# JKc66/CircuitVision

Hardware: AMD Instinct MI355X
Metric: circuit images/sec (YOLOv11 640² + SAM2.1-L 1024²) at 1/2/4/8 MI355X (higher is better)
Workload: dtype f16; 1 GPU; YOLO11-n 640x640 batch=32 f16 forward+decode+NMS (BASELINE configs[1]) + SAM2.1 Hiera-L 1024x1024 2 x batch=16 f16 learned-prompt wrapper forward (configs[2]) on the same images, per GPU and step; nc=62, weights=seeded random (SAM: LoRA merged), streams=3

## Files before the change

circuitvision_amd/_lib.py:

```python
import ctypes as C
import os

_HERE = os.path.dirname(os.path.abspath(__file__))
LIB_PATH = os.environ.get("CVMI_LIB_PATH") or os.path.join(_HERE, "libcvmi355.so")

F16, F32, BF16 = 0, 1, 2
ACT_NONE, ACT_SILU, ACT_RELU, ACT_GELU, ACT_SIGMOID = 0, 1, 2, 3, 4


class CvmiError(RuntimeError):
    pass


class ConvDesc(C.Structure):
    _fields_ = [
        ("x0", C.c_void_p), ("x1", C.c_void_p), ("w", C.c_void_p), ("bias", C.c_void_p),
        ("res", C.c_void_p), ("y", C.c_void_p),
        ("x0_ld", C.c_int), ("x1_ld", C.c_int), ("res_ld", C.c_int), ("y_ld", C.c_int),
        ("c0", C.c_int), ("c1", C.c_int), ("up0", C.c_int), ("up1", C.c_int),
        ("B", C.c_int), ("H", C.c_int), ("W", C.c_int), ("OH", C.c_int), ("OW", C.c_int),
        ("KH", C.c_int), ("KW", C.c_int), ("stride", C.c_int), ("pad", C.c_int),
        ("N", C.c_int), ("Kpad", C.c_int), ("act", C.c_int), ("dtype", C.c_int),
        ("out_f32", C.c_int), ("scalar_gather", C.c_int),
        ("res_mod", C.c_int), ("act_after_res", C.c_int), ("shuffle_cout", C.c_int), ("res_rep", C.c_int),
        ("row_stats", C.c_void_p),
    ]


class C3k2Desc(C.Structure):
    _fields_ = [
        ("x", C.c_void_p), ("y", C.c_void_p),
        ("w0", C.c_void_p), ("w1", C.c_void_p), ("w2", C.c_void_p), ("w3", C.c_void_p),
        ("b0", C.c_void_p), ("b1", C.c_void_p), ("b2", C.c_void_p), ("b3", C.c_void_p),
        ("x_ld", C.c_int), ("y_ld", C.c_int), ("kpad0", C.c_int), ("kpad1", C.c_int), ("kpad2", C.c_int), ("kpad3", C.c_int),
        ("B", C.c_int), ("H", C.c_int), ("W", C.c_int), ("c1", C.c_int), ("c", C.c_int), ("h", C.c_int), ("c2", C.c_int),
        ("fuse_cv1", C.c_int), ("shortcut", C.c_int), ("dtype", C.c_int),
    ]


class DwPwDesc(C.Structure):
    _fields_ = [
        ("x", C.c_void_p), ("y", C.c_void_p), ("wd", C.c_void_p), ("bd", C.c_void_p),
        ("w1", C.c_void_p), ("b1", C.c_void_p), ("w2", C.c_void_p), ("b2", C.c_void_p),
        ("x_ld", C.c_int), ("y_ld", C.c_int), ("kpad1", C.c_int), ("kpad2", C.c_int),
        ("B", C.c_int), ("H", C.c_int), ("W", C.c_int), ("C", C.c_int), ("N1", C.c_int), ("N2", C.c_int),
        ("dtype", C.c_int),
    ]


class AttnDesc(C.Structure):
    _fields_ = [
        ("q", C.c_void_p), ("k", C.c_void_p), ("v", C.c_void_p), ("o", C.c_void_p),
        ("q_sb", C.c_longlong), ("q_sh", C.c_longlong), ("q_st", C.c_longlong),
        ("k_sb", C.c_longlong), ("k_sh", C.c_longlong), ("k_st", C.c_longlong),
        ("v_sb", C.c_longlong), ("v_sh", C.c_longlong), ("v_st", C.c_longlong),
        ("o_sb", C.c_longlong), ("o_sh", C.c_longlong), ("o_st", C.c_longlong),
        ("B", C.c_int), ("heads", C.c_int), ("Nq", C.c_int), ("Nk", C.c_int),
        ("dqk", C.c_int), ("dv", C.c_int), ("scale", C.c_float), ("dtype", C.c_int),
        ("win", C.c_int), ("grid_h", C.c_int), ("grid_w", C.c_int), ("q_pool", C.c_int),
        ("q_bdiv", C.c_int), ("kv_bdiv", C.c_int), ("av_fp8", C.c_int), ("q_log2", C.c_int),
        ("proj_x", C.c_void_p), ("proj_w", C.c_void_p), ("proj_gamma", C.c_void_p), ("proj_beta", C.c_void_p), ("proj_stats", C.c_void_p),
        ("proj_ld", C.c_int), ("proj_K", C.c_int), ("proj_eps", C.c_float),
    ]


class LetterboxRow(C.Structure):
    _fields_ = [("src_byte_offset", C.c_longlong), ("H", C.c_int), ("W", C.c_int), ("new_h", C.c_int), ("new_w", C.c_int), ("top", C.c_int), ("left", C.c_int)]


class Sam2SrcRow(C.Structure):
    _fields_ = [("src_byte_offset", C.c_longlong), ("H", C.c_int), ("W", C.c_int), ("x0", C.c_int), ("y0", C.c_int), ("w", C.c_int), ("h", C.c_int)]


LETTERBOX_ROW = [(n, "<i8" if t is C.c_longlong else "<i4") for n, t in LetterboxRow._fields_]
SAM2_SRC_ROW = [(n, "<i8" if t is C.c_longlong else "<i4") for n, t in Sam2SrcRow._fields_]


_vp, _i, _f = C.c_void_p, C.c_int, C.c_float
SIGNATURES = {
    "cvmi_version": (_i, []),
    "cvmi_last_error": (C.c_char_p, []),
    "cvmi_last_kernel": (C.c_char_p, []),
    "cvmi_device_info": (_i, [_i, C.POINTER(_i)]),
    "cvmi_desc_size": (C.c_size_t, [_i]),
    "cvmi_graph_begin": (_i, [_vp]),
    "cvmi_graph_end": (_i, [_vp, C.POINTER(_vp)]),
    "cvmi_graph_launch": (_i, [_vp, _vp]),
    "cvmi_graph_destroy": (_i, [_vp]),
    "cvmi_conv2d": (_i, [C.POINTER(ConvDesc), _vp]),
    "cvmi_c3k2_supported": (_i, [_i, _i, _i, _i, _i, _i]),
    "cvmi_c3k2": (_i, [C.POINTER(C3k2Desc), _vp]),
    "cvmi_stem2_supported": (_i, [_i, _i, _i]),
    "cvmi_stem2": (_i, [_vp, _i, _vp, _vp, _i, _vp, _vp, _i, _vp, _i, _i, _i, _i, _i, _i, _i, _vp]),
    "cvmi_dwpw_supported": (_i, [_i, _i, _i, _i]),
    "cvmi_dwpw": (_i, [C.POINTER(DwPwDesc), _vp]),
    "cvmi_dwconv3x3": (_i, [_vp, _i, _vp, _vp, _vp, _i, _vp, _i, _i, _i, _i, _i, _i, _i, _vp]),
    "cvmi_sppf_pool": (_i, [_vp, _i, _i, _i, _i, _i, _i, _vp]),
    "cvmi_attention": (_i, [C.POINTER(AttnDesc), _vp]),
    "cvmi_detect_decode": (_i, [C.POINTER(_vp), C.POINTER(_i), C.POINTER(_vp), C.POINTER(_i), C.POINTER(_i),
                                C.POINTER(_i), C.POINTER(_f), _i, _i, _i, _i, _vp, _vp, _vp, _i, _vp]),
    "cvmi_yolo_nms_best": (_i, [_vp, _vp, _vp, _i, _i, _i, _f, _f, _i, _f, _vp, _vp, _vp, _vp, _vp]),
    "cvmi_yolo_nms_workspace": (C.c_size_t, [_i, _i]),
    "cvmi_yolo_nms": (_i, [_vp, _i, _i, _i, _f, _f, _i, _f, _vp, _vp, _vp, _vp, _vp]),
    "cvmi_letterbox": (_i, [_vp, _i, _i, _vp, _i, _i, _i, _i, _i, _i, _i, _i, _vp]),
    "cvmi_letterbox_batch": (_i, [_vp, _i, _i, _i, _vp, C.c_longlong, _i, _i, _i, _i, _i, _i, _i, _i, _vp]),
    "cvmi_letterbox_ragged": (_i, [_vp, C.c_longlong, _vp, _i, _vp, C.c_longlong, _i, _i, _i, _i, _vp]),
    "cvmi_nchw_to_nhwc": (_i, [_vp, _i, _vp, _i, _i, _i, _i, _i, _i, _vp]),
    "cvmi_nhwc_to_nchw_f32": (_i, [_vp, _i, _i, _vp, _i, _i, _i, _i, _vp]),
    "cvmi_layernorm": (_i, [_vp, _i, _i, _vp, _vp, _vp, _i, _i, C.c_longlong, _i, _f, _i, _i, _i, _i, _i, _vp]),
    "cvmi_layernorm_dual": (_i, [_vp, _i, _vp, _vp, _vp, _i, _vp, _i, _i, C.c_longlong, _i, _f, _vp]),
    "cvmi_hiera_mlp_supported": (_i, [_i]),
    "cvmi_hiera_mlp_packed_bytes": (C.c_size_t, [_i]),
    "cvmi_hiera_mlp": (_i, [_vp, _i, _vp, _vp, _f, _vp, _vp, C.c_longlong, _i, _i, _vp]),
    "cvmi_hiera_mlp_stats": (_i, [_vp, _i, _vp, _vp, _f, _vp, _vp, C.c_longlong, _i, _i, _vp, _f, _vp]),
    "cvmi_tok_linear_supported": (_i, [_i]),
    "cvmi_tok_linear_packed_bytes": (C.c_size_t, [_i, _i]),
    "cvmi_tok_linear_format": (_i, [_i]),
    "cvmi_tok_linear_stats_parts": (_i, [C.c_longlong, _i, _i]),
    "cvmi_tok_linear": (_i, [_vp, _i, _i, _vp, _vp, _f, _vp, _vp, _i, _i, C.c_longlong, _i, _i, _i, _i, _vp]),
    "cvmi_tok_linear_stats": (_i, [_vp, _i, _i, _vp, _vp, _f, _vp, _vp, _i, _i, C.c_longlong, _i, _i, _i, _i, _vp, _i, _vp, _f, _vp]),
    "cvmi_tok_linear_pool_stats": (_i, [_vp, _i, _vp, _vp, _f, _vp, _vp, _i, _i, _i, _i, _i, _i, _i, _vp, _vp]),
    "cvmi_tok_linear_pool": (_i, [_vp, _i, _vp, _vp, _f, _vp, _vp, _i, _i, _i, _i, _i, _i, _i, _vp]),
    "cvmi_maxpool2x2": (_i, [_vp, _i, _vp, _i, _i, _i, _i, _i, _i, _vp]),
    "cvmi_space_to_depth4": (_i, [_vp, _vp, _i, _i, _i, _i, _vp]),
    "cvmi_cast": (_i, [_vp, _i, _i, _vp, _i, _i, C.c_longlong, _i, _vp]),
    "cvmi_prompt_tokens": (_i, [_vp, _vp, _vp, _vp, _vp, _f, _vp, _vp, _i, _i, _i, _i, _vp]),
    "cvmi_repeat_images": (_i, [_vp, _vp, C.c_longlong, _i, _i, _vp]),
    "cvmi_hyper_masks": (_i, [_vp, _i, _vp, _i, _i, _i, _vp, _vp, _i, _i, _f, _vp]),
    "cvmi_select_mask": (_i, [_vp, _vp, _vp, _i, _i, _f, _vp, _vp, _vp, _i, _i, _vp]),
    "cvmi_multimask_out": (_i, [_vp, _vp, _i, _vp, _vp, _i, _i, _vp]),
    "cvmi_mask_prompt_embed": (_i, [_vp, _vp, _vp, _vp, _vp, _i, _i, _i, _i, _vp]),
    "cvmi_bilinear_f32": (_i, [_vp, _i, _i, _i, _vp, _i, _i, _vp, _f, _vp]),
    "cvmi_mask_extent": (_i, [_vp, _i, _i, _i, _vp, _vp]),
    "cvmi_mask_postprocess": (_i, [_vp, _i, _i, _i, _i, _i, _f, _vp, _vp, _vp]),
    "cvmi_mask_postprocess_sizes": (_i, [_vp, _i, _i, _i, _vp, _f, _vp, _vp, _vp]),
    "cvmi_mask_cc_workspace": (C.c_size_t, [_i, _i, _i]),
    "cvmi_mask_components": (_i, [_vp, _i, _i, _i, _f, _vp, _vp, _vp, _vp]),
    "cvmi_mask_fill_small": (_i, [_vp, _i, _i, _i, _f, _f, _f, _vp, _vp, _vp]),
    "cvmi_node_prepare": (_i, [_vp, _i, _vp, _vp, _vp, _vp, _vp, _vp]),
    "cvmi_enhance_lines": (_i, [_vp, _i, _vp, _vp, _vp, _vp]),
    "cvmi_contours_workspace": (C.c_size_t, [_i, _vp]),
    "cvmi_external_contours": (_i, [_vp, _vp, _i, _vp, _i, _vp, C.c_size_t, _i, _i, _vp, _vp, _vp, _vp, _vp]),
    "cvmi_node_connect_workspace": (C.c_size_t, [_i, _i]),
    "cvmi_node_connect": (_i, [_vp, _vp, _i, _i, _vp, _i, _vp, _vp, _vp, C.c_size_t, _vp, _vp, _vp]),
    "cvmi_segment_circuit": (_i, [_vp, C.c_size_t, _i, _vp, _i, _vp, _vp, _vp, _vp, _vp]),
    "cvmi_contour_hits_workspace": (C.c_size_t, [_i, _i]),
    "cvmi_contour_hits": (_i, [_vp, _vp, _i, _i, _vp, _i, _vp, _vp, _vp, C.c_size_t, _vp, _vp]),
    "cvmi_upsample_refine": (_i, [_vp, _i, _i, _i, _vp, _i, _i, _vp, C.POINTER(_i), _i, _i, _vp]),
    "cvmi_sam2_transform": (_i, [_vp, _i, _i, _vp, _i, _i, _vp]),
    "cvmi_sam2_transform_batch": (_i, [_vp, _i, _i, _i, _vp, _i, _i, _i, _vp]),
    "cvmi_sam2_transform_rects": (_i, [_vp, C.c_longlong, _i, _i, _vp, _i, _vp, _i, _i, _i, _vp]),
    "cvmi_sam2_transform_rects_dev": (_i, [_vp, C.c_longlong, _i, _i, _vp, _i, _vp, _i, _i, _i, _vp]),
    "cvmi_sam2_transform_srcs": (_i, [_vp, C.c_longlong, _vp, _i, _vp, _i, _i, _i, _vp]),
    "cvmi_mask_postprocess_rects_dev": (_i, [_vp, _i, _i, _i, _vp, C.c_longlong, _f, _vp, _vp, _vp]),
    "cvmi_stage2_crop": (_i, [_vp, _vp, _i, _i, _i, _i, _f, _i, _i, C.c_double, _i, _vp, _i, _vp, _vp, _vp, _vp, _vp, _vp, _vp]),
}

_lib = None


def load():
    global _lib
    if _lib is not None:
        return _lib
    if not os.path.exists(LIB_PATH):
        raise CvmiError(
            f"{LIB_PATH} not found: build it with `python -c 'import __graft_entry__ as g; g.build()'` "
            "(or `make -C circuitvision_amd/csrc`).  There is no CPU fallback.")
    import torch
    lib = C.CDLL(LIB_PATH)
    for name, (res, args) in SIGNATURES.items():
        fn = getattr(lib, name)
        fn.restype = res
        fn.argtypes = args
    check_abi(lib)
    _lib = lib
    return lib


DESC_MIRRORS = {0: ConvDesc, 1: C3k2Desc, 2: DwPwDesc, 3: AttnDesc}


def check_abi(lib, mirrors=None):
    for kind, cls in (mirrors or DESC_MIRRORS).items():
        want = int(lib.cvmi_desc_size(kind))
        if want != C.sizeof(cls):
            raise CvmiError(f"ABI mismatch: {cls.__name__} is {C.sizeof(cls)} bytes in this binding but {want} bytes in {LIB_PATH} "
                            f"(cvmi_desc_size({kind})); rebuild the library or update the binding to include/cvmi355.h")


def check(rc, what=""):
    if rc != 0:
        msg = load().cvmi_last_error().decode("utf-8", "replace")
        raise CvmiError(f"{what or 'cvmi call'} failed: {msg}")
```

circuitvision_amd/csrc/hiera_mlp.hip:

```cpp
#include "tok_stream.hpp"
#include <stdlib.h>

namespace {

#ifdef CVMI_OPERAND_BF16
#define CVMI_MFMA_ASM "v_mfma_f32_32x32x16_bf16"
#else
#define CVMI_MFMA_ASM "v_mfma_f32_32x32x16_f16"
#endif

template <int N1, int NT> constexpr int stage_frag(int i) { return i < N1 ? 2 * NT + i : (i - N1 < NT ? 2 * (i - N1) : 2 * (i - N1 - NT) + 1); }

template <int I, int N, typename F> __device__ __forceinline__ void static_for(F&& f) {
  if constexpr (I < N) {
    f(std::integral_constant<int, I>{});
    static_for<I + 1, N>(f);
  }
}

template <int C, int VAR = 0> struct MlpCfg {
  static_assert((C == 144 && VAR == 1) || (C == 288 && (VAR == 0 || VAR == 2)), "the instances that are built");
  static constexpr int KS = C / 16;
  static constexpr int KS1 = KS + 1;
  static constexpr int NT = (C + 31) / 32;
  static constexpr int NCH = 4 * C / 32;
  static constexpr int FR = KS1 + 2 * NT;
  static constexpr int CHB = FR * 1024;
  static constexpr int NW = 4;
  static constexpr int WPS = VAR == 1 ? 2 : 1;
  static constexpr int SLOTS = 2;
  static constexpr int CNT = (FR + NW - 1) / NW;
  static constexpr int LDS = SLOTS * CHB + 1024;
};

template <int C, int VAR = 0>
__global__ __launch_bounds__((MlpCfg<C, VAR>::NW * 64), (MlpCfg<C, VAR>::WPS)) void hiera_mlp_kernel(float* __restrict__ x, int x_ld, const float* __restrict__ gamma,
                                                                                      const float* __restrict__ beta, float eps,
                                                                                      const char* __restrict__ wp, const float* __restrict__ b2,
                                                                                      long long rows, float* __restrict__ stats_out, float stats_eps) {
  using Cfg = MlpCfg<C, VAR>;
  constexpr int KS = Cfg::KS, KS1 = Cfg::KS1, NT = Cfg::NT, NCH = Cfg::NCH, FR = Cfg::FR, CHB = Cfg::CHB, NW = Cfg::NW, CNT = Cfg::CNT, SLOTS = Cfg::SLOTS;
  extern __shared__ __attribute__((aligned(16))) char smem[];
  const int tid = threadIdx.x, wv = __builtin_amdgcn_readfirstlane(tid >> 6), lane = tid & 63;
  const int lr = lane & 31, lh = lane >> 5;
  const long long row_raw = ((long long)blockIdx.x * NW + wv) * 32 + lr;
  const bool row_ok = row_raw < rows;
  float* const xr = x + (row_ok ? row_raw : rows - 1) * (long long)x_ld;

  auto issue_chunk = [&](int j) {
    const char* src = wp + (size_t)j * CHB + lane * 16;
    char* dst = smem + (j % SLOTS) * CHB;
#pragma unroll
    for (int f = 0; f < CNT; ++f) {
      const int fi = f * NW + wv;
      const bool real = fi < FR;
      __builtin_amdgcn_global_load_lds((const __attribute__((address_space(1))) void*)(src + (size_t)(real ? fi : 0) * 1024),
                                       (__attribute__((address_space(3))) void*)(real ? dst + fi * 1024 : smem + SLOTS * CHB), 16, 0, 0);
    }
  };
  auto issue_piece = [&](int st, int f) {
    const int lo = st < 0 ? 2 * NT : 0, hi = st == NCH - 1 ? 2 * NT : FR;
    const char* src = wp + ((long long)st * FR + KS1) * 1024 + lane * 16;
    char* dst = smem + ((st + SLOTS) % SLOTS) * CHB;
    const int fi = f * NW + wv;
    const bool real = fi >= lo && fi < hi;
    __builtin_amdgcn_global_load_lds((const __attribute__((address_space(1))) void*)(src + (long long)(real ? fi : lo) * 1024),
                                     (__attribute__((address_space(3))) void*)(real ? dst + fi * 1024 : smem + SLOTS * CHB), 16, 0, 0);
  };
  auto issue_stage = [&](int st) {
#pragma unroll
    for (int f = 0; f < CNT; ++f) issue_piece(st, f);
  };
  if constexpr (VAR == 2) {
#pragma unroll
    for (int st = -1; st < SLOTS - 1; ++st) issue_stage(st);
  } else {
#pragma unroll
    for (int j = 0; j < SLOTS - 1; ++j) issue_chunk(j);
  }

  u32x4 xn[KS1];
  {
    float v[KS][8];
    float s = 0.f;
#pragma unroll
    for (int k = 0; k < KS; ++k) {
      const f32x4 a = *reinterpret_cast<const f32x4*>(xr + 16 * k + 8 * lh), b = *reinterpret_cast<const f32x4*>(xr + 16 * k + 8 * lh + 4);
#pragma unroll
      for (int e = 0; e < 4; ++e) { v[k][e] = a[e]; v[k][4 + e] = b[e]; s += a[e] + b[e]; }
    }
    s += __shfl_xor(s, 32);
    const float mean = s / (float)C;
    float q = 0.f;
#pragma unroll
    for (int k = 0; k < KS; ++k)
#pragma unroll
      for (int e = 0; e < 8; ++e) { const float d = v[k][e] - mean; q += d * d; }
    q += __shfl_xor(q, 32);
    const float rstd = 1.0f / sqrtf(q / (float)C + eps);
#pragma unroll
    for (int k = 0; k < KS; ++k) {
      const float* gp = gamma + 16 * k + 8 * lh;
      const float* bp = beta + 16 * k + 8 * lh;
      const f32x4 g0 = *reinterpret_cast<const f32x4*>(gp), g1 = *reinterpret_cast<const f32x4*>(gp + 4);
      const f32x4 b0 = *reinterpret_cast<const f32x4*>(bp), b1 = *reinterpret_cast<const f32x4*>(bp + 4);
      f16x8 h;
#pragma unroll
      for (int e = 0; e < 4; ++e) {
        h[e] = (f16)((v[k][e] - mean) * rstd * g0[e] + b0[e]);
        h[4 + e] = (f16)((v[k][4 + e] - mean) * rstd * g1[e] + b1[e]);
      }
      xn[k] = __builtin_bit_cast(u32x4, h);
    }
    const u32x4 one = {lh == 0 ? CVMI_ONE16X2 : 0u, 0u, 0u, 0u};
    xn[KS] = one;
  }

  f32x16 yacc[NT];
#pragma unroll
  for (int t = 0; t < NT; ++t)
#pragma unroll
    for (int r = 0; r < 16; ++r) yacc[t][r] = 0.f;

  if constexpr (VAR == 2) {
    static_assert(SLOTS == 2, "two stages in LDS");
    constexpr int PF = 6;
    f32x16 hA, hB;
    u32x4 ring_[PF];
#pragma unroll
    for (int f = 0; f < PF; ++f) asm volatile("" : "=v"(ring_[f]));
#pragma unroll
    for (int k = 0; k < KS1; ++k) asm volatile("s_nop 1" : "+v"(xn[k]));
    GeluPk2Steps gs[4];
    u32x4 pfv[2] = {};
    uint32_t c1v = GeluPk2Steps::GELU_C1_H;
    asm volatile("" : "+v"(c1v));
    auto gelu_step = [&](f32x16& h, auto kc) {
      constexpr int k = decltype(kc)::value, c = k >> 2;
      GeluPk2Steps& g = gs[c];
      if constexpr ((k & 3) == 0) g.s0(h[4 * c], h[4 * c + 1], h[4 * c + 2], h[4 * c + 3]);
      else if constexpr ((k & 3) == 1) g.s1(c1v);
      else if constexpr ((k & 3) == 2) g.s2();
      else {
        g.s3();
        pfv[c >> 1][2 * (c & 1)] = g.ra;
        pfv[c >> 1][2 * (c & 1) + 1] = g.rb;
      }
    };
    auto iter = [&](auto mode_, int slot, f32x16& hin, f32x16& hout) {
      constexpr int MODE = decltype(mode_)::value;
      constexpr int N1 = MODE == 2 ? 0 : KS1, N2 = MODE == 0 ? 0 : 2 * NT, NF = N1 + N2;
      const unsigned lbase_ = (unsigned)(size_t)((const __attribute__((address_space(3))) char*)(smem + slot * CHB + lane * 16));
      static_for<0, PF>([&](auto fc) {
        constexpr int f = decltype(fc)::value;
        u32x4(&ring)[PF] = ring_;
        const unsigned lbase = lbase_;
        asm volatile("ds_read_b128 %0, %1 offset:%2" : "+v"(ring[f]) : "v"(lbase), "n"(stage_frag<N1, NT>(f) * 1024));
      });
      if constexpr (MODE != 0) asm volatile("" : "+v"(hin));
      static_for<0, NF>([&](auto ic) {
        constexpr int i = decltype(ic)::value;
        u32x4(&ring)[PF] = ring_;
        const unsigned lbase = lbase_;
        f32x16 &hi_ = hin, &ho_ = hout;
        u32x4(&pfw)[2] = pfv;
        u32x4(&xf)[KS1] = xn;
        f32x16(&ya)[NT] = yacc;
        constexpr int young = (NF - 1 - i) < (PF - 1) ? (NF - 1 - i) : (PF - 1);
        constexpr bool refill = i + PF < NF;
        constexpr int off = refill ? stage_frag<N1, NT>(i + PF) * 1024 : 0;
        if constexpr (i == N1 && MODE != 0) asm volatile("s_nop 1" : "+v"(pfw[0]));
        if constexpr (i == N1 + NT && MODE != 0) asm volatile("s_nop 1" : "+v"(pfw[1]));
#define CVMI_MLP_BLK(TAIL, ACCC, ACC, B)                                                                                                              \
  if constexpr (refill)                                                                                                                                \
    asm volatile("s_waitcnt lgkmcnt(%[n])\n\t" CVMI_MFMA_ASM " %[acc], %[a], %[b], " TAIL "\n\tds_read_b128 %[a], %[lb] offset:%[off]"               \
                 : [acc] ACCC(ACC), [a] "+v"(ring[i % PF]) : [b] "v"(B), [lb] "v"(lbase), [n] "n"(young), [off] "n"(off));                             \
  else                                                                                                                                                 \
    asm volatile("s_waitcnt lgkmcnt(%[n])\n\t" CVMI_MFMA_ASM " %[acc], %[a], %[b], " TAIL : [acc] ACCC(ACC), [a] "+v"(ring[i % PF]) : [b] "v"(B), [n] "n"(young))
        if constexpr (i < N1) {
          if constexpr (i == 0) { CVMI_MLP_BLK("0", "=&v", ho_, xf[i]); }
          else { CVMI_MLP_BLK("%[acc]", "+v", ho_, xf[i]); }
        } else {
          constexpr int t = (i - N1) % NT, s2 = (i - N1) / NT;
          CVMI_MLP_BLK("%[acc]", "+a", ya[t], pfw[s2]);
        }
#undef CVMI_MLP_BLK
        constexpr int SL = MODE == 1 ? N1 + NT : NT, K0 = MODE == 1 ? 0 : 8;
        if constexpr (MODE != 0 && i < SL)
          static_for<K0, 16>([&](auto kc) {
            if constexpr ((decltype(kc)::value - K0) * SL / (16 - K0) == i) gelu_step(hi_, kc);
          });
      });
    };
    asm volatile("s_waitcnt vmcnt(%0)" ::"n"((SLOTS - 1) * CNT) : "memory");
    __syncthreads();
    iter(std::integral_constant<int, 0>{}, SLOTS - 1, hA, hA);
    auto step = [&](auto mode, int j, f32x16& hin, f32x16& hout) {
      asm volatile("s_waitcnt vmcnt(0)" ::: "memory");
      __syncthreads();
      if (j + 1 < NCH) issue_stage(j + 1);
      iter(mode, j % SLOTS, hin, hout);
    };
    static_assert(NCH % 2 == 0, "pairs of iterations");
#pragma unroll 1
    for (int j = 0; j < NCH - 2; j += 2) {
      step(std::integral_constant<int, 1>{}, j, hA, hB);
      step(std::integral_constant<int, 1>{}, j + 1, hB, hA);
    }
    step(std::integral_constant<int, 1>{}, NCH - 2, hA, hB);
    {
      asm volatile("s_waitcnt vmcnt(0)" ::: "memory");
      __syncthreads();
      asm volatile("" : "+v"(hB));
      static_for<0, 8>([&](auto kc) { gelu_step(hB, kc); });
      iter(std::integral_constant<int, 2>{}, (NCH - 1) % SLOTS, hB, hB);
    }
#pragma unroll
    for (int t = 0; t < NT; ++t) asm volatile("s_nop 15" : "+a"(yacc[t]));
#pragma unroll
    for (int f = 0; f < PF; ++f) asm volatile("" ::"v"(ring_[f]));
  } else
#pragma unroll 1
  for (int j = 0; j < NCH; ++j) {
    asm volatile("s_waitcnt vmcnt(0)" ::: "memory");
    __syncthreads();
    if (j + SLOTS - 1 < NCH) issue_chunk(j + SLOTS - 1);
    const char* const buf = smem + (j % SLOTS) * CHB + lane * 16;
    constexpr int PF = 6;
    u32x4 ring[PF];
    const unsigned lbase = (unsigned)(size_t)((const __attribute__((address_space(3))) char*)buf);
#pragma unroll
    for (int f = 0; f < PF; ++f) asm volatile("ds_read_b128 %0, %1 offset:%2" : "=v"(ring[f]) : "v"(lbase), "i"(f * 1024));
    f32x16 hacc;
#pragma unroll
    for (int r = 0; r < 16; ++r) hacc[r] = 0.f;
    f16x8 pf[2];
#pragma unroll
    for (int f = 0; f < FR; ++f) {
      ring_wait(ring[f % PF], (FR - 1 - f) < (PF - 1) ? (FR - 1 - f) : (PF - 1));
      const f16x8 a = __builtin_bit_cast(f16x8, ring[f % PF]);
      if (f < KS1) {
        hacc = CVMI_MFMA_32X32X16(a, __builtin_bit_cast(f16x8, xn[f]), hacc, 0, 0, 0);
      } else {
        const int t = (f - KS1) >> 1, s2 = (f - KS1) & 1;
        yacc[t] = CVMI_MFMA_32X32X16(a, pf[s2], yacc[t], 0, 0, 0);
      }
      if (f + PF < FR) asm volatile("ds_read_b128 %0, %1 offset:%2" : "=v"(ring[f % PF]) : "v"(lbase), "i"((f + PF) * 1024));
      if (f == KS1 - 1) {
#pragma unroll
        for (int r = 0; r < 16; r += 2) {
          const f16x2 g2 = gelu_fast_pk(hacc[r], hacc[r + 1]);
          pf[r >> 3][r & 7] = g2[0];
          pf[r >> 3][(r & 7) + 1] = g2[1];
        }
      }
    }
  }

  ShiftedSums st;
  if (stats_out) {
    const float o0 = row_ok ? xr[0] + (yacc[0][0] + b2[0]) : 0.f;
    st.shift = __shfl(o0, lr);
  }
  if (row_ok) {
#pragma unroll
    for (int t = 0; t < NT; ++t)
#pragma unroll
      for (int g = 0; g < 4; ++g) {
        const int c0 = 32 * t + 8 * g + 4 * lh;
        if (c0 < C) {
          const f32x4 bb = *reinterpret_cast<const f32x4*>(b2 + c0);
          f32x4 o = *reinterpret_cast<const f32x4*>(xr + c0);
#pragma unroll
          for (int e = 0; e < 4; ++e) o[e] += yacc[t][4 * g + e] + bb[e];
          *reinterpret_cast<f32x4*>(xr + c0) = o;
          if (stats_out) st.add(o);
        }
      }
  }
  if (stats_out) {
    const float2 mr = shifted_mean_rstd(st.shift, row_sum<2>(st.s), row_sum<2>(st.q), (float)C, stats_eps);
    if (row_ok && lh == 0) *reinterpret_cast<float2*>(stats_out + 2 * row_raw) = mr;
  }
}

template <int C, int VAR = 0>
int launch_mlp(float* x, int x_ld, const float* gamma, const float* beta, float eps, const void* wp, const float* b2, long long rows, hipStream_t s,
               float* stats_out, float stats_eps) {
  using Cfg = MlpCfg<C, VAR>;
  static hipError_t attr = hipFuncSetAttribute(reinterpret_cast<const void*>(&hiera_mlp_kernel<C, VAR>), hipFuncAttributeMaxDynamicSharedMemorySize, Cfg::LDS);
  CVMI_HIP(attr);
  const long long per = (long long)Cfg::NW * 32;
  cvmi_note_kernel("hiera_mlp_kernel<%d, %d>", C, VAR);
  hipLaunchKernelGGL((hiera_mlp_kernel<C, VAR>), dim3((unsigned)((rows + per - 1) / per)), dim3(Cfg::NW * 64), Cfg::LDS, s, x, x_ld, gamma, beta, eps,
                     (const char*)wp, b2, rows, stats_out, stats_eps);
  CVMI_LAUNCH_CHECK();
  return 0;
}

}

#ifndef CVMI_OPERAND_BF16
extern "C" int cvmi_hiera_mlp_supported(int C) { return C == 144 || C == 288; }

extern "C" size_t cvmi_hiera_mlp_packed_bytes(int C) {
  if (!cvmi_hiera_mlp_supported(C)) return 0;
  const size_t fr = (size_t)(C / 16 + 1) + 2 * (size_t)((C + 31) / 32);
  return (size_t)(4 * C / 32) * fr * 1024;
}
extern "C" int cvmi_hiera_mlp_stats_bf16(void* x, int x_ld, const float* gamma, const float* beta, float eps, const void* w_packed, const float* b2,
                                         long long rows, int C, int dtype, float* ln_stats_out, float ln_stats_eps, cvmi_stream_t stream_);
#endif

extern "C" int CVMI_ENTRY(cvmi_hiera_mlp_stats)(void* x, int x_ld, const float* gamma, const float* beta, float eps, const void* w_packed, const float* b2,
                                                long long rows, int C, int dtype, float* ln_stats_out, float ln_stats_eps, cvmi_stream_t stream_) {
#ifndef CVMI_OPERAND_BF16
  if (dtype == CVMI_BF16) return cvmi_hiera_mlp_stats_bf16(x, x_ld, gamma, beta, eps, w_packed, b2, rows, C, dtype, ln_stats_out, ln_stats_eps, stream_);
#endif
  CVMI_CHECK(dtype == CVMI_T16, "hiera_mlp: dtype must be CVMI_F16 or CVMI_BF16");
  CVMI_CHECK(x && gamma && beta && w_packed && b2 && rows > 0, "hiera_mlp: bad arguments");
  CVMI_CHECK(C == 144 || C == 288, "hiera_mlp: C=%d is not built (144, 288)", C);
  CVMI_CHECK(x_ld >= C && x_ld % 4 == 0 && (((uintptr_t)x | (uintptr_t)gamma | (uintptr_t)beta | (uintptr_t)w_packed | (uintptr_t)b2) & 15) == 0 &&
                 ((uintptr_t)ln_stats_out & 7) == 0,
             "hiera_mlp: pointers / ld must be 16-byte aligned");
  hipStream_t s = (hipStream_t)stream_;
  float* xf = (float*)x;
  if (C == 144) return launch_mlp<144, 1>(xf, x_ld, gamma, beta, eps, w_packed, b2, rows, s, ln_stats_out, ln_stats_eps);
  const char* const pipe = getenv("CVMI_MLP_PIPE");
  if (pipe && !(atoi(pipe) & 2)) return launch_mlp<288, 0>(xf, x_ld, gamma, beta, eps, w_packed, b2, rows, s, ln_stats_out, ln_stats_eps);
  return launch_mlp<288, 2>(xf, x_ld, gamma, beta, eps, w_packed, b2, rows, s, ln_stats_out, ln_stats_eps);
}

extern "C" int CVMI_ENTRY(cvmi_hiera_mlp)(void* x, int x_ld, const float* gamma, const float* beta, float eps, const void* w_packed, const float* b2,
                                          long long rows, int C, int dtype, cvmi_stream_t stream_) {
  return CVMI_ENTRY(cvmi_hiera_mlp_stats)(x, x_ld, gamma, beta, eps, w_packed, b2, rows, C, dtype, nullptr, 0.f, stream_);
}
```

circuitvision_amd/engine.py:

```python
import ctypes as C
import os
import threading

import torch

from . import _lib
from ._lib import BF16, F16, F32, AttnDesc, C3k2Desc, ConvDesc

TORCH_DTYPE = {F16: torch.float16, F32: torch.float32, BF16: torch.bfloat16}
ESIZE = {F16: 2, F32: 4, BF16: 2}
DTYPE_OF = {torch.float16: F16, torch.float32: F32, torch.bfloat16: BF16}


def is16(dtype):
    return dtype in (F16, BF16)


def require_gpu():
    if not torch.cuda.is_available():
        raise _lib.CvmiError("circuitvision_amd needs an MI355X (gfx950) GPU: torch.cuda.is_available() is False; "
                             "there is no CPU fallback")
    _lib.load()


class Buf:

    def __init__(self, B, H, W, C, dtype, device="cuda", zero=False):
        self.B, self.H, self.W, self.C, self.dtype = B, H, W, C, dtype
        alloc = torch.zeros if zero else torch.empty
        self.t = alloc((B, H, W, C), dtype=TORCH_DTYPE[dtype], device=device)

    def view(self, c0=0, c=None):
        return View(self, c0, self.C - c0 if c is None else c)

    def images(self, b0, nb):
        assert 0 <= b0 and b0 + nb <= self.B
        o = Buf.__new__(Buf)
        o.B, o.H, o.W, o.C, o.dtype = nb, self.H, self.W, self.C, self.dtype
        o.t = self.t[b0:b0 + nb]
        return o

    @property
    def nbytes(self):
        return self.t.numel() * self.t.element_size()


class View:

    def __init__(self, buf, c0, c):
        assert 0 <= c0 and c0 + c <= buf.C, (c0, c, buf.C)
        self.buf, self.c0, self.c = buf, c0, c

    @property
    def ptr(self):
        return self.buf.t.data_ptr() + self.c0 * ESIZE[self.buf.dtype]

    @property
    def ld(self):
        return self.buf.C

    B = property(lambda s: s.buf.B)
    H = property(lambda s: s.buf.H)
    W = property(lambda s: s.buf.W)
    dtype = property(lambda s: s.buf.dtype)

    def tensor(self):
        return self.buf.t[..., self.c0:self.c0 + self.c]


class PackedConv:

    def __init__(self, weight, bias, dtype, device="cuda"):
        N, Cin, KH, KW = weight.shape
        K = Cin * KH * KW
        Npad = (N + 127) // 128 * 128
        Kpad = (K + 63) // 64 * 64
        w = torch.zeros(Npad, Kpad, dtype=torch.float32)
        w[:N, :K] = weight.permute(0, 2, 3, 1).reshape(N, K)
        b = torch.zeros(Npad, dtype=torch.float32)
        if bias is not None:
            b[:N] = bias
        self.w = w.to(TORCH_DTYPE[dtype]).to(device)
        self.bias = b.to(device)
        self.N, self.Cin, self.KH, self.KW, self.K, self.Kpad, self.dtype = N, Cin, KH, KW, K, Kpad, dtype
        self.param_bytes = N * K * ESIZE[dtype]


class PackedDW:

    def __init__(self, weight, bias, dtype, device="cuda"):
        C_ = weight.shape[0]
        assert weight.shape[1:] == (1, 3, 3)
        self.w = weight.reshape(C_, 9).t().contiguous().to(TORCH_DTYPE[dtype]).to(device)
        self.bias = (bias if bias is not None else torch.zeros(C_)).float().to(device)
        self.C, self.dtype = C_, dtype
        self.param_bytes = C_ * 9 * ESIZE[dtype]


class Plan:

    def __init__(self, stream):
        self.stream = stream
        self.ops = []
        self.keep = []
        self.graph = None
        self.lanes, self.cur_lane = [], 0
        self._lane_streams = {}
        self._lock = threading.Lock()

    @property
    def sptr(self):
        return self.stream.cuda_stream

    def add(self, label, kind, thunk, bytes_=0, flops=0):
        self.ops.append((label, kind, thunk, bytes_, flops))
        self.lanes.append(self.cur_lane)

    def fork(self):
        self.add("fork", "sync", lambda sp=None: None)
        self.lanes[-1] = -1

    def lane(self, i):
        self.cur_lane = i

    def join(self):
        self.cur_lane = 0
        self.add("join", "sync", lambda sp=None: None)
        self.lanes[-1] = -2

    def run_eager(self):
        for _, _, thunk, _, _ in self.ops:
            thunk()

    def capture(self):
        lib = _lib.load()
        self.run_eager()
        self.stream.synchronize()
        _lib.check(lib.cvmi_graph_begin(self.sptr), "graph_begin")
        try:
            self._run_lanes()
        finally:
            g = C.c_void_p()
            rc = lib.cvmi_graph_end(self.sptr, C.byref(g))
        _lib.check(rc, "graph_end")
        self.graph = g

    def _run_lanes(self):
        active, lane_fork = {}, {}
        for (label, kind, thunk, _, _), lane in zip(self.ops, self.lanes):
            if lane == -1:
                self._fork_ev = torch.cuda.Event()
                self._fork_ev.record(self.stream)
            elif lane == -2:
                for st in active.values():
                    ev = torch.cuda.Event()
                    ev.record(st)
                    self.stream.wait_event(ev)
                active, lane_fork = {}, {}
            elif lane == 0:
                thunk()
            else:
                if lane not in self._lane_streams:
                    self._lane_streams[lane] = torch.cuda.Stream(device=self.stream.device)
                st = self._lane_streams[lane]
                if lane_fork.get(lane) is not self._fork_ev:
                    st.wait_event(self._fork_ev)
                    lane_fork[lane] = self._fork_ev
                    active[lane] = st
                thunk(st.cuda_stream)

    def run(self):
        if self.graph is None:
            self.capture()
        _lib.check(_lib.load().cvmi_graph_launch(self.graph, self.sptr), "graph_launch")

    def timed_eager(self, with_kernels=False):
        lib = _lib.load()
        lib.cvmi_last_kernel()
        evs = []
        for label, kind, thunk, b, f in self.ops:
            e0 = torch.cuda.Event(enable_timing=True)
            e1 = torch.cuda.Event(enable_timing=True)
            e0.record(self.stream)
            thunk()
            e1.record(self.stream)
            evs.append((label, kind, e0, e1, b, f, lib.cvmi_last_kernel().decode()))
        self.stream.synchronize()
        if with_kernels:
            return [(l, k, e0.elapsed_time(e1), b, f, kn) for l, k, e0, e1, b, f, kn in evs]
        return [(l, k, e0.elapsed_time(e1), b, f) for l, k, e0, e1, b, f, _ in evs]

    def __del__(self):
        try:
            if self.graph is not None:
                if self._lane_streams or os.environ.get("CVMI_KEEP_GRAPHS") == "1":
                    _PARKED_GRAPHS.append((self.graph, self._lane_streams))
                else:
                    _lib.load().cvmi_graph_destroy(self.graph)
        except Exception:
            pass


_PARKED_GRAPHS = []


def row_stats_supported(M, N, K):
    if N % 192 or N < 384 or K < 1024 or K % 64:
        return False
    t256 = -(-M // 256) * -(-N // 256)
    if t256 >= 256 and N / (-(-N // 256) * 256) >= 0.8 and t256 / (-(-t256 // 256) * 256) >= 0.8:
        return False
    t192 = -(-M // 256) * (N // 192)
    return t192 >= 256 and t192 / (-(-t192 // 256) * 256) >= 0.75


def op_conv(plan, label, pc, srcs, dst, stride=1, pad=None, act=_lib.ACT_NONE, res=None, out_hw=None,
            scalar_gather=False, kind="conv", res_mod=0, act_after_res=False, shuffle_cout=0, res_rep=0, row_stats=None):
    lib = _lib.load()
    (v0, up0) = srcs[0]
    v1, up1 = (srcs[1] if len(srcs) > 1 else (None, 0))
    H, W = v0.H << up0, v0.W << up0
    if v1 is not None:
        assert (v1.H << up1, v1.W << up1) == (H, W), "concatenated sources disagree on size"
    ctot = v0.c + (v1.c if v1 is not None else 0)
    assert ctot == pc.Cin, (label, ctot, pc.Cin)
    pad = pc.KH // 2 if pad is None else pad
    OH = (H + 2 * pad - pc.KH) // stride + 1
    OW = (W + 2 * pad - pc.KW) // stride + 1
    if out_hw is not None:
        assert out_hw[0] <= OH and out_hw[1] <= OW
        OH, OW = out_hw
    if shuffle_cout:
        assert (dst.B, dst.H, dst.W) == (v0.B, 2 * OH, 2 * OW) and dst.c == shuffle_cout and pc.N == 4 * shuffle_cout, label
    else:
        assert (dst.B, dst.H, dst.W) == (v0.B, OH, OW) and dst.c == pc.N, (label, (dst.B, dst.H, dst.W, dst.c), (v0.B, OH, OW, pc.N))
    if res_rep > 1:
        assert res is not None and res.B * res_rep == v0.B, (label, "res_rep needs a per-image residual")
        assert shuffle_cout or res_mod == dst.H * dst.W, (label, "res_rep: ConvTranspose scatter or res_mod = rows per image")
    out_f32 = 1 if (dst.dtype == F32 and is16(pc.dtype)) else 0
    d = ConvDesc(
        x0=v0.ptr, x1=(v1.ptr if v1 is not None else None), w=pc.w.data_ptr(), bias=pc.bias.data_ptr(),
        res=(res.ptr if res is not None else None), y=dst.ptr,
        x0_ld=v0.ld, x1_ld=(v1.ld if v1 is not None else 0), res_ld=(res.ld if res is not None else 0), y_ld=dst.ld,
        c0=v0.c, c1=(v1.c if v1 is not None else 0), up0=up0, up1=up1,
        B=v0.B, H=H, W=W, OH=OH, OW=OW, KH=pc.KH, KW=pc.KW, stride=stride, pad=pad,
        N=pc.N, Kpad=pc.Kpad, act=act, dtype=pc.dtype, out_f32=out_f32, scalar_gather=1 if scalar_gather else 0,
        res_mod=res_mod, act_after_res=1 if act_after_res else 0, shuffle_cout=shuffle_cout, res_rep=res_rep,
        row_stats=(row_stats.data_ptr() if row_stats is not None else None))
    if row_stats is not None:
        assert row_stats.dtype == torch.float32 and row_stats.is_contiguous() and row_stats.numel() == v0.B * OH * OW * (pc.N // 96) * 2, label
    plan.keep.append((d, pc, srcs, dst, res, row_stats))
    sp0 = plan.sptr
    fn = lib.cvmi_conv2d

    def thunk(sp=None):
        sp = sp0 if sp is None else sp
        _lib.check(fn(C.byref(d), sp), label)

    M = v0.B * OH * OW
    es, oes = ESIZE[pc.dtype], ESIZE[dst.dtype]
    in_elems = v0.B * (v0.H * v0.W * v0.c + (v1.H * v1.W * v1.c if v1 is not None else 0))
    bytes_ = in_elems * es + M * pc.N * oes + (M * pc.N * oes if res is not None else 0)
    plan.add(label, kind, thunk, bytes_, 2 * M * pc.N * pc.K)
    return d


def c3k2_supported(c1, c, h, c2, fuse_cv1, dtype):
    return bool(_lib.load().cvmi_c3k2_supported(c1, c, h, c2, 1 if fuse_cv1 else 0, dtype))


def op_c3k2(plan, label, src, dst, pc_cv1, pc_m1, pc_m2, pc_cv2, c, h, fuse_cv1, shortcut=True):
    lib = _lib.load()
    assert (src.B, src.H, src.W) == (dst.B, dst.H, dst.W) and dst.c == pc_cv2.N
    assert src.c == (pc_cv1.Cin if fuse_cv1 else 2 * c), (label, src.c)
    d = C3k2Desc(x=src.ptr, y=dst.ptr, w0=pc_cv1.w.data_ptr() if fuse_cv1 else None, w1=pc_m1.w.data_ptr(), w2=pc_m2.w.data_ptr(),
                 w3=pc_cv2.w.data_ptr(), b0=pc_cv1.bias.data_ptr() if fuse_cv1 else None, b1=pc_m1.bias.data_ptr(), b2=pc_m2.bias.data_ptr(),
                 b3=pc_cv2.bias.data_ptr(), x_ld=src.ld, y_ld=dst.ld, kpad0=pc_cv1.Kpad if fuse_cv1 else 0, kpad1=pc_m1.Kpad, kpad2=pc_m2.Kpad,
                 kpad3=pc_cv2.Kpad, B=src.B, H=src.H, W=src.W, c1=pc_cv1.Cin if fuse_cv1 else 0, c=c, h=h, c2=pc_cv2.N,
                 fuse_cv1=1 if fuse_cv1 else 0, shortcut=1 if shortcut else 0, dtype=pc_cv2.dtype)
    plan.keep.append((d, src, dst, pc_cv1, pc_m1, pc_m2, pc_cv2))
    sp0, fn = plan.sptr, lib.cvmi_c3k2

    def thunk(sp=None):
        sp = sp0 if sp is None else sp
        _lib.check(fn(C.byref(d), sp), label)

    px = src.B * src.H * src.W
    flops = 2 * px * ((pc_cv1.Cin * 2 * c if fuse_cv1 else 0) + 9 * c * h * 2 + 3 * c * pc_cv2.N)
    plan.add(label, "conv", thunk, px * (src.c + dst.c) * ESIZE[pc_cv2.dtype], flops)


def stem2_supported(c0, c1, dtype):
    return bool(_lib.load().cvmi_stem2_supported(c0, c1, dtype))


def op_stem2(plan, label, pc0, pc1, src, dst):
    lib = _lib.load()
    assert src.c == 16 and pc0.Cin == 16 and pc1.Cin == pc0.N and dst.c == pc1.N
    assert (dst.H, dst.W) == ((src.H - 1) // 2 + 1, (src.W - 1) // 2 + 1) and dst.B == src.B
    args = (src.ptr, src.ld, pc0.w.data_ptr(), pc0.bias.data_ptr(), pc0.Kpad, pc1.w.data_ptr(), pc1.bias.data_ptr(), pc1.Kpad,
            dst.ptr, dst.ld, src.B, src.H, src.W, pc0.N, pc1.N, pc1.dtype)
    plan.keep.append((pc0, pc1, src, dst))
    sp0, fn = plan.sptr, lib.cvmi_stem2

    def thunk(sp=None):
        sp = sp0 if sp is None else sp
        _lib.check(fn(*args, sp), label)

    px0, px1 = src.B * src.H * src.W, dst.B * dst.H * dst.W
    plan.add(label, "stem", thunk, (px0 * src.c + px1 * dst.c) * ESIZE[pc1.dtype], 2 * px0 * 27 * pc0.N + 2 * px1 * 9 * pc0.N * pc1.N)


def dwpw_supported(C_, n1, n2, dtype):
    return bool(_lib.load().cvmi_dwpw_supported(C_, n1, n2, dtype))


def op_dwpw(plan, label, pd, pc1, src, dst, pc2=None):
    lib = _lib.load()
    assert src.c == pd.C == pc1.Cin and (src.B, src.H, src.W) == (dst.B, dst.H, dst.W)
    assert dst.c == (pc2.N if pc2 is not None else pc1.N) and (pc2 is None or pc2.Cin == pc1.N)
    d = _lib.DwPwDesc(x=src.ptr, y=dst.ptr, wd=pd.w.data_ptr(), bd=pd.bias.data_ptr(), w1=pc1.w.data_ptr(), b1=pc1.bias.data_ptr(),
                      w2=pc2.w.data_ptr() if pc2 is not None else None, b2=pc2.bias.data_ptr() if pc2 is not None else None,
                      x_ld=src.ld, y_ld=dst.ld, kpad1=pc1.Kpad, kpad2=pc2.Kpad if pc2 is not None else 0,
                      B=src.B, H=src.H, W=src.W, C=pd.C, N1=pc1.N, N2=pc2.N if pc2 is not None else 0, dtype=pc1.dtype)
    plan.keep.append((d, pd, pc1, pc2, src, dst))
    sp0, fn = plan.sptr, lib.cvmi_dwpw

    def thunk(sp=None):
        sp = sp0 if sp is None else sp
        _lib.check(fn(C.byref(d), sp), label)

    px = src.B * src.H * src.W
    flops = px * (18 * pd.C + 2 * pd.C * pc1.N + (2 * pc1.N * pc2.N if pc2 is not None else 0))
    plan.add(label, "head", thunk, px * (src.c + dst.c) * ESIZE[pc1.dtype], flops)


def op_dwconv(plan, label, pd, src, dst, act=_lib.ACT_NONE, res=None):
    lib = _lib.load()
    assert src.c == pd.C == dst.c and (src.B, src.H, src.W) == (dst.B, dst.H, dst.W)
    args = (src.ptr, src.ld, pd.w.data_ptr(), pd.bias.data_ptr(), res.ptr if res is not None else None,
            res.ld if res is not None else 0, dst.ptr, dst.ld, src.B, src.H, src.W, pd.C, act, pd.dtype)
    plan.keep.append((pd, src, dst, res))
    sp0 = plan.sptr
    fn = lib.cvmi_dwconv3x3

    def thunk(sp=None):
        sp = sp0 if sp is None else sp
        _lib.check(fn(*args, sp), label)

    n = src.B * src.H * src.W * pd.C
    plan.add(label, "dwconv", thunk, n * ESIZE[pd.dtype] * (3 if res is not None else 2), 18 * n)


def op_sppf_pool(plan, label, buf, c):
    lib = _lib.load()
    args = (buf.t.data_ptr(), buf.C, buf.B, buf.H, buf.W, c, buf.dtype)
    plan.keep.append(buf)
    sp0 = plan.sptr
    fn = lib.cvmi_sppf_pool

    def thunk(sp=None):
        sp = sp0 if sp is None else sp
        _lib.check(fn(*args, sp), label)

    n = buf.B * buf.H * buf.W * c
    plan.add(label, "pool", thunk, 4 * n * ESIZE[buf.dtype], 0)


def op_attention(plan, label, desc, keep, bytes_=0, flops=0):
    lib = _lib.load()
    plan.keep.append((desc, keep))
    sp0 = plan.sptr
    fn = lib.cvmi_attention

    def thunk(sp=None):
        sp = sp0 if sp is None else sp
        _lib.check(fn(C.byref(desc), sp), label)

    plan.add(label, "attention", thunk, bytes_, flops)


def make_attn_desc(**kw):
    d = AttnDesc()
    for k, v in kw.items():
        setattr(d, k, v)
    return d


class Rows:

    def __init__(self, t, rows, C, ld=None, offset=0, dtype=None):
        self.t, self.rows, self.C = t, rows, C
        self.ld = ld if ld is not None else C
        self.offset = offset
        self.dtype = dtype if dtype is not None else DTYPE_OF[t.dtype]

    @property
    def ptr(self):
        return self.t.data_ptr() + self.offset * self.t.element_size()


def op_layernorm(plan, label, src, gamma, beta, dst, eps=1e-6, act=_lib.ACT_NONE, pad=None, dst2=None):
    lib = _lib.load()
    src, dst = _as_rows(src), _as_rows(dst)
    assert src.C == dst.C == gamma.numel()
    if dst2 is not None:
        dst2 = _as_rows(dst2)
        assert pad is None and act == _lib.ACT_NONE and src.dtype == dst.dtype == _lib.F32 and is16(dst2.dtype)
        assert dst2.rows == src.rows and dst2.C == src.C
        args2 = (src.ptr, src.ld, gamma.data_ptr(), beta.data_ptr(), dst.ptr, dst.ld, dst2.ptr, dst2.ld, dst2.dtype, src.rows, src.C, float(eps))
        plan.keep.append((src, dst, dst2, gamma, beta))
        sp1, fn2 = plan.sptr, lib.cvmi_layernorm_dual

        def thunk2(sp=None):
            sp = sp1 if sp is None else sp
            _lib.check(fn2(*args2, sp), label)

        plan.add(label, "layernorm", thunk2, src.rows * src.C * (4 + 4 + 2), 8 * src.rows * src.C)
        return
    if pad is None:
        assert src.rows == dst.rows
        pad = (0, 0, 0, 0)
    else:
        assert src.rows % (pad[0] * pad[1]) == 0 and dst.rows == src.rows // (pad[0] * pad[1]) * pad[2] * pad[3]
    args = (src.ptr, src.ld, src.dtype, gamma.data_ptr(), beta.data_ptr(), dst.ptr, dst.ld, dst.dtype, src.rows, src.C, float(eps), act) + tuple(pad)
    plan.keep.append((src, dst, gamma, beta))
    sp0, fn = plan.sptr, lib.cvmi_layernorm

    def thunk(sp=None):
        sp = sp0 if sp is None else sp
        _lib.check(fn(*args, sp), label)

    plan.add(label, "layernorm", thunk, src.rows * src.C * (ESIZE[src.dtype] + ESIZE[dst.dtype]), 8 * src.rows * src.C)


def _as_rows(v):
    if isinstance(v, Rows):
        return v
    if isinstance(v, View):
        return Rows(v.buf.t, v.B * v.H * v.W, v.c, ld=v.ld, offset=v.c0, dtype=v.dtype)
    raise TypeError(type(v))


def op_maxpool2(plan, label, src, dst):
    lib = _lib.load()
    assert src.c == dst.c and (dst.H, dst.W) == (src.H // 2, src.W // 2) and src.dtype == dst.dtype
    args = (src.ptr, src.ld, dst.ptr, dst.ld, src.B, src.H, src.W, src.c, src.dtype)
    plan.keep.append((src, dst))
    sp0, fn = plan.sptr, lib.cvmi_maxpool2x2

    def thunk(sp=None):
        sp = sp0 if sp is None else sp
        _lib.check(fn(*args, sp), label)

    n = src.B * src.H * src.W * src.c
    plan.add(label, "pool", thunk, n * ESIZE[src.dtype] * 5 // 4, 0)


def op_cast(plan, label, src, dst):
    lib = _lib.load()
    src, dst = _as_rows(src), _as_rows(dst)
    args = (src.ptr, src.ld, src.dtype, dst.ptr, dst.ld, dst.dtype, src.rows, src.C)
    plan.keep.append((src, dst))
    sp0, fn = plan.sptr, lib.cvmi_cast

    def thunk(sp=None):
        sp = sp0 if sp is None else sp
        _lib.check(fn(*args, sp), label)

    plan.add(label, "cast", thunk, src.rows * src.C * (ESIZE[src.dtype] + ESIZE[dst.dtype]), 0)


def op_call(plan, label, kind, fn, args, keep=(), bytes_=0, flops=0):
    plan.keep.append(keep)
    sp0 = plan.sptr

    def thunk(sp=None):
        sp = sp0 if sp is None else sp
        _lib.check(fn(*args, sp), label)

    plan.add(label, kind, thunk, bytes_, flops)


def hiera_mlp_supported(C_, dtype):
    return is16(dtype) and bool(_lib.load().cvmi_hiera_mlp_supported(C_))


class PackedHieraMlp:

    def __init__(self, w1, b1, w2, b2, device="cuda", dtype=F16):
        td = TORCH_DTYPE[dtype]
        Hd, C_ = w1.shape
        assert Hd == 4 * C_ and tuple(w2.shape) == (C_, Hd) and C_ % 16 == 0
        ks1, nt, nch = C_ // 16 + 1, (C_ + 31) // 32, Hd // 32
        b_hi = b1.to(td).float()
        b_lo = (b1 - b_hi).to(td).float()
        w1x = torch.cat((w1, b_hi[:, None], b_lo[:, None], torch.zeros(Hd, 14)), 1)
        f1 = w1x.view(nch, 32, ks1, 2, 8).permute(0, 2, 3, 1, 4)
        w2p = torch.zeros(nt * 32, Hd)
        w2p[:C_] = w2
        f2 = w2p.view(nt, 32, nch, 2, 2, 2, 4).permute(2, 0, 3, 5, 1, 4, 6)
        packed = torch.cat((f1.reshape(nch, -1), f2.reshape(nch, -1)), 1).contiguous()
        assert packed.numel() * 2 == _lib.load().cvmi_hiera_mlp_packed_bytes(C_)
        self.w = packed.to(td).to(device)
        self.bias = b2.float().contiguous().to(device)
        self.C, self.dtype = C_, dtype
        self.param_bytes = 2 * Hd * C_ * 2


def op_hiera_mlp(plan, label, pm, x, gamma, beta, eps=1e-6, stats_out=None, stats_eps=1e-6):
    lib = _lib.load()
    assert x.dtype == F32 and x.c == pm.C and x.c0 == 0
    rows = x.B * x.H * x.W
    assert stats_out is None or (stats_out.dtype == torch.float32 and stats_out.numel() == 2 * rows and stats_out.is_contiguous()), label
    args = (x.ptr, x.ld, gamma.data_ptr(), beta.data_ptr(), float(eps), pm.w.data_ptr(), pm.bias.data_ptr(), rows, pm.C, pm.dtype,
            stats_out.data_ptr() if stats_out is not None else None, float(stats_eps))
    plan.keep.append((pm, x, gamma, beta, stats_out))
    sp0, fn = plan.sptr, lib.cvmi_hiera_mlp_stats

    def thunk(sp=None):
        sp = sp0 if sp is None else sp
        _lib.check(fn(*args, sp), label)

    plan.add(label, "mlp_fused", thunk, rows * pm.C * 8, 2 * rows * 2 * 4 * pm.C * pm.C)


def tok_linear_supported(K, dtype, rows):
    return is16(dtype) and rows % 256 == 0 and bool(_lib.load().cvmi_tok_linear_supported(K))


class PackedTokLinear:

    def __init__(self, w, b, device="cuda", dtype=F16):
        N, K = w.shape
        td = TORCH_DTYPE[dtype]
        assert K % 16 == 0
        if _lib.load().cvmi_tok_linear_format(K) == 16:
            nch, ks = (N + 31) // 32, K // 32
            b = b if b is not None else torch.zeros(N)
            wx = torch.zeros(nch * 32, K)
            wx[:N] = w
            frag = wx.view(nch, 2, 16, ks, 4, 8).permute(0, 3, 1, 4, 2, 5).reshape(nch, ks * 2 * 512)
            bias = torch.zeros(nch * 32)
            bias[:N] = b
            piece = torch.zeros(nch, 512, dtype=torch.int16)
            piece[:, :64] = bias.view(nch, 32).contiguous().view(torch.int16)
            packed = torch.cat((frag.to(td).contiguous().view(torch.int16), piece), 1).contiguous()
            assert packed.numel() * 2 == _lib.load().cvmi_tok_linear_packed_bytes(K, N)
            self.w = packed.to(device)
            self.bias = torch.zeros(4, device=device)
            self.N, self.K, self.dtype = N, K, dtype
            self.param_bytes = N * K * 2
            return
        ks1, nch = K // 16 + 1, ((N + 31) // 32 + 1) // 2 * 2
        b = b if b is not None else torch.zeros(N)
        b_hi = b.to(td).float()
        b_lo = (b - b_hi).to(td).float()
        wx = torch.zeros(nch * 32, K + 16)
        wx[:N, :K], wx[:N, K], wx[:N, K + 1] = w, b_hi, b_lo
        packed = wx.view(nch, 32, ks1, 2, 8).permute(0, 2, 3, 1, 4).contiguous()
        assert packed.numel() * 2 == _lib.load().cvmi_tok_linear_packed_bytes(K, N)
        self.w = packed.to(td).to(device)
        self.bias = torch.zeros(4, device=device)
        self.N, self.K, self.dtype = N, K, dtype
        self.param_bytes = N * K * 2


def qkv_attn_rows(heads, hd=72):
    C_ = heads * hd
    rows = []
    for h in range(heads):
        for c in range(3):
            for r in range(32):
                g, lh, e = r >> 3, (r >> 2) & 1, r & 3
                d = 32 * c + 16 * (g >> 1) + 8 * lh + 4 * (g & 1) + e
                rows.append(h * hd + d if d < hd else -1)
        rows += [C_ + h * hd + n if n < hd else 2 * C_ + h * hd + n - hd if n < 2 * hd else -1 for n in range(160)]
    return rows


def qkv_attn_supported(dim, dout, heads, ws, q_pool, dtype, nwin):
    return is16(dtype) and dim == 144 and ws == 8 and nwin % 2 == 0 and (dout, heads) == ((288, 4) if q_pool else (144, 2))


class PackedQkvAttn:

    def __init__(self, w, b, heads, device="cuda", dtype=F16):
        N, K = w.shape
        assert N % (3 * heads) == 0
        self.rows = qkv_attn_rows(heads, N // (3 * heads))
        idx = torch.tensor(self.rows)
        keep = (idx >= 0).float()
        b = b if b is not None else torch.zeros(N)
        pt = PackedTokLinear(w[idx.clamp(min=0)] * keep[:, None], b[idx.clamp(min=0)] * keep, device, dtype)
        self.w, self.bias = pt.w, pt.bias
        self.N, self.K, self.heads, self.dtype = N, K, heads, dtype
        self.param_bytes = pt.param_bytes


def tok_linear_stats_parts(rows, K, N):
    return int(_lib.load().cvmi_tok_linear_stats_parts(rows, K, N))


def op_tok_linear(plan, label, pt, src, dst, ln=None, act=_lib.ACT_NONE, residual=False, kind="gemm", stats_in=None, stats_out=None, stats_eps=1e-6,
                  stats_parts=0):
    lib = _lib.load()
    src, dst = _as_rows(src), _as_rows(dst)
    assert src.C == pt.K and dst.C == pt.N and src.rows == dst.rows and src.rows % 256 == 0, label
    assert (src.dtype == F32) == (ln is not None) and (dst.dtype == F32) == bool(residual), label
    assert (ln is not None or src.dtype == pt.dtype) and (residual or dst.dtype == pt.dtype), label
    cast = isinstance(ln, str)
    assert not cast or ln == "cast", label
    assert stats_in is None or (ln is not None and not cast), label
    assert stats_out is None or residual, label
    out_parts = tok_linear_stats_parts(src.rows, pt.K, pt.N) if stats_out is not None else 0
    assert stats_out is None or (stats_out.dtype == torch.float32 and stats_out.numel() == 2 * src.rows * max(out_parts, 1) and stats_out.is_contiguous()), label
    assert stats_in is None or (stats_in.dtype == torch.float32 and stats_in.numel() == 2 * src.rows * max(stats_parts, 1) and stats_in.is_contiguous()), label
    gam, bet, eps = ln if (ln is not None and not cast) else (None, None, 0.0)
    args = (src.ptr, src.ld, 2 if cast else 1 if ln is not None else 0, gam.data_ptr() if gam is not None else None, bet.data_ptr() if bet is not None else None,
            float(eps), pt.w.data_ptr(), dst.ptr, dst.ld, 1 if residual else 0, src.rows, pt.K, pt.N, act, pt.dtype,
            stats_in.data_ptr() if stats_in is not None else None, int(stats_parts), stats_out.data_ptr() if stats_out is not None else None, float(stats_eps))
    plan.keep.append((pt, src, dst, gam, bet, stats_in, stats_out))
    sp0, fn = plan.sptr, lib.cvmi_tok_linear_stats

    def thunk(sp=None):
        sp = sp0 if sp is None else sp
        _lib.check(fn(*args, sp), label)

    bytes_ = src.rows * (pt.K * ESIZE[src.dtype] + pt.N * ESIZE[dst.dtype] * (2 if residual else 1))
    plan.add(label, kind, thunk, bytes_, 2 * src.rows * pt.N * pt.K)


def op_tok_linear_pool(plan, label, pt, src, dst, ln, kind="gemm", stats_in=None):
    lib = _lib.load()
    B, H, W = src.B, src.H, src.W
    assert src.dtype == F32 and dst.dtype == F32 and src.c == pt.K and dst.c == pt.N, label
    assert (dst.B, dst.H, dst.W) == (B, H // 2, W // 2) and H % 2 == 0 and W % 2 == 0 and (B * H * W) % 256 == 0, label
    gam, bet, eps = ln
    assert stats_in is None or (stats_in.dtype == torch.float32 and stats_in.numel() == 2 * B * H * W and stats_in.is_contiguous()), label
    args = (src.ptr, src.ld, gam.data_ptr(), bet.data_ptr(), float(eps), pt.w.data_ptr(), dst.ptr, dst.ld, B, H, W, pt.K, pt.N, pt.dtype,
            stats_in.data_ptr() if stats_in is not None else None)
    plan.keep.append((pt, src, dst, gam, bet, stats_in))
    sp0, fn = plan.sptr, lib.cvmi_tok_linear_pool_stats

    def thunk(sp=None):
        sp = sp0 if sp is None else sp
        _lib.check(fn(*args, sp), label)

    rows = B * H * W
    plan.add(label, kind, thunk, rows * pt.K * 4 + rows // 4 * pt.N * 4, 2 * rows * pt.N * pt.K)
```

circuitvision_amd/sam2.py:

```python
import hashlib
import math
import os
import threading

import numpy as np
import torch
import torch.nn.functional as TF

from . import _lib
from ._lib import ACT_GELU, ACT_NONE, ACT_RELU, ACT_SIGMOID, BF16, F16, F32
from .engine import (ESIZE, TORCH_DTYPE, is16, Buf, PackedConv, PackedHieraMlp, PackedQkvAttn, PackedTokLinear, Plan, Rows, hiera_mlp_supported, make_attn_desc, op_attention,
                     op_call, op_cast, op_conv, op_hiera_mlp, op_layernorm, op_maxpool2, op_tok_linear, op_tok_linear_pool, require_gpu, row_stats_supported,
                     qkv_attn_supported, tok_linear_stats_parts, tok_linear_supported)

LOG2E = 1.4426950408889634
HIERA_L = dict(embed_dim=144, num_heads=2, stages=(2, 6, 36, 4), global_att_blocks=(23, 33, 43), window_spec=(8, 4, 16, 8))
HIERA_T = dict(embed_dim=96, num_heads=1, stages=(1, 2, 7, 2), global_att_blocks=(5, 7, 9), window_spec=(8, 4, 14, 7))

LORA_TARGETS_REFERENCE = (
    [f"sam_mask_decoder.transformer.layers.{l}.{a}.{p}" for l in (0, 1) for a in ("self_attn", "cross_attn_token_to_image")
     for p in ("k_proj", "q_proj", "v_proj", "out_proj")]
    + [f"sam_mask_decoder.transformer.layers.{l}.mlp.layers.{j}" for l in (0, 1) for j in (0, 1)]
    + ["sam_mask_decoder.iou_prediction_head.layers.2", "sam_mask_decoder.conv_s0", "sam_mask_decoder.conv_s1",
       "image_encoder.neck.convs.2.conv", "image_encoder.neck.convs.3.conv",
       "image_encoder.trunk.blocks.44.attn.qkv", "image_encoder.trunk.blocks.44.mlp.layers.0", "image_encoder.trunk.blocks.44.proj",
       "image_encoder.trunk.blocks.47.attn.qkv", "image_encoder.trunk.blocks.47.mlp.layers.0"]
    + [f"sam_mask_decoder.transformer.layers.{l}.cross_attn_image_to_token.{p}" for l in (0, 1) for p in ("q_proj", "k_proj", "v_proj")])


MASK_DOWN = "sam_prompt_encoder.mask_downscaling"
MASK_DOWN_PARAMS = 4684


def mask_down_tensors():
    return [(f"{MASK_DOWN}.0.weight", (4, 1, 2, 2), "w"), (f"{MASK_DOWN}.0.bias", (4,), "w"),
            (f"{MASK_DOWN}.1.weight", (4,), "gamma"), (f"{MASK_DOWN}.1.bias", (4,), "w"),
            (f"{MASK_DOWN}.3.weight", (16, 4, 2, 2), "w"), (f"{MASK_DOWN}.3.bias", (16,), "w"),
            (f"{MASK_DOWN}.4.weight", (16,), "gamma"), (f"{MASK_DOWN}.4.bias", (16,), "w"),
            (f"{MASK_DOWN}.6.weight", (256, 16, 1, 1), "w"), (f"{MASK_DOWN}.6.bias", (256,), "w")]


class SamSyntheticParams:

    def __init__(self, seed=0, lora_targets=LORA_TARGETS_REFERENCE, r=4, alpha=16, std=0.02):
        self.seed, self.targets, self.r, self.scaling, self.std, self.sd = seed, set(lora_targets), r, alpha / r, std, {}
        self.mask_sd = {}

    def _t(self, name, shape, kind="w"):
        sd = self.mask_sd if name.startswith(MASK_DOWN + ".") else self.sd
        if name in sd:
            assert tuple(sd[name].shape) == tuple(shape), (name, sd[name].shape, shape)
            return sd[name]
        h = int.from_bytes(hashlib.sha256(f"{self.seed}:{name}".encode()).digest()[:8], "little") & 0x7FFFFFFFFFFFFFFF
        g = torch.Generator().manual_seed(h)
        if kind == "gamma":
            t = torch.empty(shape).uniform_(0.8, 1.2, generator=g)
        elif kind == "unit":
            t = torch.empty(shape).normal_(0, 1.0, generator=g)
        elif kind == "refine":
            t = torch.empty(shape).normal_(0, 0.2, generator=g)
        else:
            t = torch.empty(shape).normal_(0, self.std, generator=g).clamp_(-2 * self.std, 2 * self.std)
        sd[name] = t
        return t

    def weight(self, mod, shape):
        if mod in self.targets:
            w = self._t(f"{mod}.base_layer.weight", shape)
            a_shape = (self.r, shape[1]) + tuple(shape[2:])
            b_shape = (shape[0], self.r) + (1,) * (len(shape) - 2)
            A = self._t(f"{mod}.lora_A.default.weight", a_shape)
            Bm = self._t(f"{mod}.lora_B.default.weight", b_shape)
            delta = (Bm.reshape(shape[0], self.r) @ A.reshape(self.r, -1)).reshape(shape)
            return w + self.scaling * delta
        return self._t(f"{mod}.weight", shape)

    def bias(self, mod, n):
        return self._t(f"{mod}.base_layer.bias" if mod in self.targets else f"{mod}.bias", (n,))

    def tensor(self, name, shape, kind="w"):
        return self._t(name, shape, kind)

    def state_dict(self):
        return dict(self.sd)

    def mask_prompt_state_dict(self):
        for name, shape, kind in mask_down_tensors():
            self._t(name, shape, kind)
        return dict(self.mask_sd)


class SamBlankParams:

    def weight(self, mod, shape):
        return torch.zeros(shape)

    def bias(self, mod, n):
        return torch.zeros(n)

    def tensor(self, name, shape, kind="w"):
        return torch.zeros(shape)

    def state_dict(self):
        return {}


class SamStateDictParams:

    PREFIXES = ("sam2_model.base_model.model.", "sam2_model.")

    def __init__(self, sd, r=4, alpha=16):
        self.scaling = alpha / r
        self.sd = {}
        for k, v in sd.items():
            for p in self.PREFIXES:
                if k.startswith(p):
                    k = k[len(p):]
                    break
            self.sd[k] = v.detach().float().cpu()

    def _get(self, name, shape):
        t = self.sd[name]
        if tuple(t.shape) != tuple(shape):
            raise ValueError(f"{name}: checkpoint shape {tuple(t.shape)} != expected {tuple(shape)}")
        return t

    def weight(self, mod, shape):
        if f"{mod}.base_layer.weight" in self.sd:
            w = self._get(f"{mod}.base_layer.weight", shape)
            A, Bm = self.sd[f"{mod}.lora_A.default.weight"], self.sd[f"{mod}.lora_B.default.weight"]
            r = A.shape[0]
            return w + self.scaling * (Bm.reshape(shape[0], r) @ A.reshape(r, -1)).reshape(shape)
        return self._get(f"{mod}.weight", shape)

    def bias(self, mod, n):
        k = f"{mod}.base_layer.bias" if f"{mod}.base_layer.bias" in self.sd else f"{mod}.bias"
        return self._get(k, (n,))

    def tensor(self, name, shape, kind="w"):
        return self._get(name, shape)


class SamBaseCheckpointParams(SamStateDictParams):

    WRAPPER = ("dense_embedding", "sparse_embedding", "refinement_layer.")

    def __init__(self, sd, seed=0):
        super().__init__(sd.get("model", sd) if isinstance(sd, dict) else sd)
        self.seed = seed

    def tensor(self, name, shape, kind="w"):
        if name in self.sd:
            return self._get(name, shape)
        if name.startswith(self.WRAPPER):
            h = int.from_bytes(hashlib.sha256(f"{self.seed}:{name}".encode()).digest()[:8], "little") & 0x7FFFFFFFFFFFFFFF
            g = torch.Generator().manual_seed(h)
            t = torch.empty(shape).normal_(0, 1.0 if "embedding" in name else 0.1, generator=g)
            self.sd[name] = t
            return t
        raise KeyError(name)


def _lin(w):
    return w.reshape(w.shape[0], w.shape[1], 1, 1)


class Sam2Weights:
    def __init__(self, params, hiera=HIERA_L, image_size=1024, dtype=F16, device="cuda", use_refinement=True,
                 refinement_kernels=(3, 5, 7, 11), embedding_r=4):
        self.p, self.hiera, self.image_size, self.dtype, self.device = params, hiera, image_size, dtype, device
        self.use_refinement, self.kernels = use_refinement, tuple(refinement_kernels)
        self.pc, self.ln, self.const, self.mlp, self.tl = {}, {}, {}, {}, {}
        self.fused_mlp = os.environ.get("CVMI_SAM_FUSED_MLP", "1") != "0"
        self.use_tok = os.environ.get("CVMI_SAM_TOKLIN", "1") != "0"
        self.q_log2 = is16(dtype) and os.environ.get("CVMI_SAM_QLOG2", "1") != "0"
        self.qkv_attn = os.environ.get("CVMI_SAM_QKVATTN", "1") != "0"
        self.param_bytes = 0
        self.flops_per_image = 0
        self._trunk()
        self._neck_and_prompts(embedding_r)
        self._decoder()
        self._refinement()

    def _pack(self, key, w4, b):
        pc = PackedConv(w4, b, self.dtype, self.device)
        self.pc[key] = pc
        self.param_bytes += pc.param_bytes
        return pc

    def _linear(self, key, mod, cout, cin, tok=False, row_scale=None, fuse_heads=0):
        w, b = self.p.weight(mod, (cout, cin)), self.p.bias(mod, cout)
        if row_scale is not None:
            n, f = row_scale
            w, b = w.clone(), b.clone()
            w[:n] *= f
            b[:n] *= f
        if tok and self.use_tok and is16(self.dtype) and tok_linear_supported(cin, self.dtype, 256):
            self.tl[key] = PackedTokLinear(w, b, self.device, self.dtype)
            if fuse_heads:
                self.tl[key + "_attn"] = PackedQkvAttn(w, b, fuse_heads, self.device, self.dtype)
        return self._pack(key, _lin(w), b)

    def _norm(self, key, mod, c):
        self.ln[key] = (self.p.tensor(f"{mod}.weight", (c,), "gamma").float().to(self.device),
                        self.p.tensor(f"{mod}.bias", (c,)).float().to(self.device))

    def _trunk(self):
        h = self.hiera
        E, stages, ws = h["embed_dim"], h["stages"], h["window_spec"]
        T = "image_encoder.trunk"
        w7 = self.p.weight(f"{T}.patch_embed.proj", (E, 3, 7, 7))
        w2 = torch.zeros(E, 48, 2, 2)
        m = {k: ((0, k + 1) if k < 3 else (1, k - 3)) for k in range(7)}
        for ky in range(7):
            for kx in range(7):
                (ty, sy), (tx, sx) = m[ky], m[kx]
                w2[:, (sy * 4 + sx) * 3:(sy * 4 + sx) * 3 + 3, ty, tx] = w7[:, :, ky, kx]
        self._pack("patch_embed", w2, self.p.bias(f"{T}.patch_embed.proj", E))
        g = self.image_size // 4
        pos = TF.interpolate(self.p.tensor(f"{T}.pos_embed", (1, E, 7, 7)), size=(g, g), mode="bicubic")
        win = self.p.tensor(f"{T}.pos_embed_window", (1, E, ws[0], ws[0]))
        pos = pos + win.tile([1, 1, g // ws[0], g // ws[0]])
        self.const["pos_embed"] = pos.permute(0, 2, 3, 1).reshape(g * g, E).contiguous().float().to(self.device)
        stage_ends = [sum(stages[:i]) - 1 for i in range(1, len(stages) + 1)]
        q_pool_blocks = [x + 1 for x in stage_ends[:-1]][:3]
        self.blocks, self.stage_ends = [], stage_ends
        cur, dim, heads = 1, E, h["num_heads"]
        for i in range(sum(stages)):
            dim_out, window = dim, ws[cur - 1]
            if i in h["global_att_blocks"]:
                window = 0
            if i - 1 in stage_ends:
                dim_out, heads, cur = dim * 2, heads * 2, cur + 1
            b = f"{T}.blocks.{i}"
            self._norm(f"b{i}.norm1", f"{b}.norm1", dim)
            self._linear(f"b{i}.qkv", f"{b}.attn.qkv", 3 * dim_out, dim, tok=True,
                         row_scale=(dim_out, (dim_out // heads) ** -0.5 * LOG2E) if self.q_log2 else None,
                         fuse_heads=heads if self.qkv_attn and qkv_attn_supported(dim, dim_out, heads, window, i in q_pool_blocks, self.dtype, 2) else 0)
            self._linear(f"b{i}.proj", f"{b}.attn.proj", dim_out, dim_out, tok=True)
            self._norm(f"b{i}.norm2", f"{b}.norm2", dim_out)
            if self.fused_mlp and hiera_mlp_supported(dim_out, self.dtype):
                self.mlp[f"b{i}"] = PackedHieraMlp(self.p.weight(f"{b}.mlp.layers.0", (4 * dim_out, dim_out)), self.p.bias(f"{b}.mlp.layers.0", 4 * dim_out),
                                                   self.p.weight(f"{b}.mlp.layers.1", (dim_out, 4 * dim_out)), self.p.bias(f"{b}.mlp.layers.1", dim_out),
                                                   self.device, self.dtype)
                self.param_bytes += self.mlp[f"b{i}"].param_bytes
            else:
                self._linear(f"b{i}.fc1", f"{b}.mlp.layers.0", 4 * dim_out, dim_out, tok=True)
                self._linear(f"b{i}.fc2", f"{b}.mlp.layers.1", dim_out, 4 * dim_out)
            if dim != dim_out:
                self._linear(f"b{i}.dimproj", f"{b}.proj", dim_out, dim, tok=True)
            self.blocks.append(dict(dim=dim, dim_out=dim_out, heads=heads, window=window, q_pool=i in q_pool_blocks))
            if window > 0 and i in q_pool_blocks and window % 2:
                raise ValueError("q-pool block with odd window")
            dim = dim_out
        self.stage_dims = [E * 2 ** s for s in range(len(stages))]

    def _neck_and_prompts(self, embedding_r):
        N, D = "image_encoder.neck", "sam_mask_decoder"
        c = self.stage_dims
        wn = [self.p.weight(f"{N}.convs.{j}.conv", (256, c[3 - j], 1, 1)).reshape(256, -1) for j in range(4)]
        bn = [self.p.bias(f"{N}.convs.{j}.conv", 256) for j in range(4)]
        ws0, bs0 = self.p.weight(f"{D}.conv_s0", (32, 256, 1, 1)).reshape(32, 256), self.p.bias(f"{D}.conv_s0", 32)
        ws1, bs1 = self.p.weight(f"{D}.conv_s1", (64, 256, 1, 1)).reshape(64, 256), self.p.bias(f"{D}.conv_s1", 64)
        self._pack("feat_s0", _lin(ws0 @ wn[3]), ws0 @ bn[3] + bs0)
        self._pack("feat_s1", _lin(ws1 @ wn[2]), ws1 @ bn[2] + bs1)
        if self.use_tok and is16(self.dtype):
            for key, w_, b_ in (("feat_s0", ws0 @ wn[3], ws0 @ bn[3] + bs0), ("feat_s1", ws1 @ wn[2], ws1 @ bn[2] + bs1)):
                if tok_linear_supported(w_.shape[1], self.dtype, 256) and w_.shape[1] <= 288:
                    self.tl[key] = PackedTokLinear(w_, b_, self.device, self.dtype)
        self._pack("embed", _lin(torch.cat((wn[1], wn[0]), 1)), bn[1] + bn[0])
        fs = self.image_size // 16
        e1 = self.p.tensor("dense_embedding1", (1, 256, embedding_r), "unit")
        e2 = self.p.tensor("dense_embedding2", (1, embedding_r, fs * fs), "unit")
        dense = (e1 @ e2).view(256, fs * fs).t().contiguous()
        self.const["dense"] = dense.float().to(self.device)
        G = self.p.tensor("sam_prompt_encoder.pe_layer.positional_encoding_gaussian_matrix", (2, 128), "unit")
        yy, xx = torch.meshgrid((torch.arange(fs, dtype=torch.float32) + 0.5) / fs, (torch.arange(fs, dtype=torch.float32) + 0.5) / fs, indexing="ij")
        cpe = 2 * math.pi * ((2 * torch.stack((xx, yy), -1) - 1) @ G)
        self.key_pe = torch.cat((torch.sin(cpe), torch.cos(cpe)), -1).reshape(fs * fs, 256)
        self.sparse = self.p.tensor("sparse_embedding", (1, 32, 256), "unit")[0]
        PE = "sam_prompt_encoder"
        try:
            table = torch.cat([self.p.tensor(f"{PE}.not_a_point_embed.weight", (1, 256), "unit")]
                              + [self.p.tensor(f"{PE}.point_embeddings.{i}.weight", (1, 256), "unit") for i in range(4)], 0)
            no_mask = self.p.tensor(f"{PE}.no_mask_embed.weight", (1, 256), "unit")[0]
            no_mem = self.p.tensor("no_mem_embed", (1, 1, 256), "unit").reshape(256)
        except KeyError:
            self.prompt_ok = self.mask_prompt_ok = False
            return
        self.prompt_ok = True
        self._pack("embed_box", _lin(torch.cat((wn[1], wn[0]), 1)), bn[1] + bn[0] + no_mask + no_mem)
        self.const["prompt_table"] = table.float().contiguous().to(self.device)
        self.const["gauss"] = G.float().contiguous().to(self.device)
        try:
            parts = [self.p.tensor(name, shape, kind).float().reshape(-1) for name, shape, kind in mask_down_tensors()]
        except KeyError:
            self.mask_prompt_ok = False
            return
        self.mask_prompt_ok = True
        parts[-1] = parts[-1] - no_mask.float()
        self.const["mask_down"] = torch.cat(parts).contiguous().to(self.device)
        assert self.const["mask_down"].numel() == MASK_DOWN_PARAMS

    def _attn(self, key, mod, inner, q_pe=None, k_pe=None):
        d = {}
        for nm in ("q_proj", "k_proj", "v_proj"):
            d[nm] = (self.p.weight(f"{mod}.{nm}", (inner, 256)), self.p.bias(f"{mod}.{nm}", inner))
        self._linear(f"{key}.out", f"{mod}.out_proj", 256, inner)
        return d

    def _decoder(self):
        D = "sam_mask_decoder"
        dev, od = self.device, TORCH_DTYPE[self.dtype]
        tokens = torch.cat((self.p.tensor(f"{D}.obj_score_token.weight", (1, 256), "unit"), self.p.tensor(f"{D}.iou_token.weight", (1, 256), "unit"),
                            self.p.tensor(f"{D}.mask_tokens.weight", (4, 256), "unit"), self.sparse), 0)
        self.tokens = tokens
        self.const["tokens"] = tokens.float().to(dev)
        kpe = self.key_pe
        self.n_tok = tokens.shape[0]
        self._sa_w, self._x_w = {}, {}

        def cres(t):
            return t.contiguous().to(od).to(dev)

        for l in (0, 1):
            L = f"{D}.transformer.layers.{l}"
            sa = self._attn(f"l{l}.sa", f"{L}.self_attn", 256)
            self._sa_w[l] = (sa["q_proj"][0], sa["k_proj"][0])
            w = torch.cat([sa[n][0] for n in ("q_proj", "k_proj", "v_proj")], 0)
            b = torch.cat([sa[n][1] for n in ("q_proj", "k_proj", "v_proj")], 0)
            self._pack(f"l{l}.sa.qkv", _lin(w), b)
            if l > 0:
                pe = torch.cat((tokens @ sa["q_proj"][0].t(), tokens @ sa["k_proj"][0].t(), torch.zeros(self.n_tok, 256)), 1)
                self.const[f"l{l}.sa.qkv_pe"] = cres(pe)
            self._norm(f"l{l}.norm1", f"{L}.norm1", 256)
            t2i = self._attn(f"l{l}.t2i", f"{L}.cross_attn_token_to_image", 128)
            self._pack(f"l{l}.t2i.q", _lin(t2i["q_proj"][0]), t2i["q_proj"][1])
            self.const[f"l{l}.t2i.q_pe"] = cres(tokens @ t2i["q_proj"][0].t())
            self._pack(f"l{l}.t2i.kv", _lin(torch.cat((t2i["k_proj"][0], t2i["v_proj"][0]), 0)), torch.cat((t2i["k_proj"][1], t2i["v_proj"][1]), 0))
            self.const[f"l{l}.t2i.kv_pe"] = cres(torch.cat((kpe @ t2i["k_proj"][0].t(), torch.zeros(kpe.shape[0], 128)), 1))
            self._norm(f"l{l}.norm2", f"{L}.norm2", 256)
            self._linear(f"l{l}.mlp1", f"{L}.mlp.layers.0", 2048, 256)
            self._linear(f"l{l}.mlp2", f"{L}.mlp.layers.1", 256, 2048)
            self._norm(f"l{l}.norm3", f"{L}.norm3", 256)
            i2t = self._attn(f"l{l}.i2t", f"{L}.cross_attn_image_to_token", 128)
            self._pack(f"l{l}.i2t.q", _lin(i2t["q_proj"][0]), i2t["q_proj"][1])
            self.const[f"l{l}.i2t.q_pe"] = cres(kpe @ i2t["q_proj"][0].t())
            self._pack(f"l{l}.i2t.kv", _lin(torch.cat((i2t["k_proj"][0], i2t["v_proj"][0]), 0)), torch.cat((i2t["k_proj"][1], i2t["v_proj"][1]), 0))
            self.const[f"l{l}.i2t.kv_pe"] = cres(torch.cat((tokens @ i2t["k_proj"][0].t(), torch.zeros(self.n_tok, 128)), 1))
            self._norm(f"l{l}.norm4", f"{L}.norm4", 256)
            self._x_w[l] = {"t2i.q": t2i["q_proj"][0], "i2t.k": i2t["k_proj"][0]}
        F_ = f"{D}.transformer.final_attn_token_to_image"
        fa = self._attn("final", F_, 128)
        zeros = lambda n: torch.zeros(n, 256)
        groups = [("l1.sa.qkv_pe", torch.cat((self._sa_w[1][0], self._sa_w[1][1], zeros(256)), 0))]
        for l in (0, 1):
            groups.append((f"l{l}.t2i.q_pe", self._x_w[l]["t2i.q"]))
            groups.append((f"l{l}.i2t.kv_pe", torch.cat((self._x_w[l]["i2t.k"], zeros(128)), 0)))
        groups.append(("final.q_pe", fa["q_proj"][0]))
        self.pe_off, off = {}, 0
        for name, w in groups:
            self.pe_off[name] = (off, w.shape[0])
            off += w.shape[0]
        self._pack("token_pe", _lin(torch.cat([w for _, w in groups], 0)), torch.zeros(off))
        self.const["out_tokens"] = tokens[:6].float().contiguous().to(dev)
        self._pack("final.q", _lin(fa["q_proj"][0]), fa["q_proj"][1])
        self.const["final.q_pe"] = cres(tokens @ fa["q_proj"][0].t())
        self._pack("final.kv", _lin(torch.cat((fa["k_proj"][0], fa["v_proj"][0]), 0)), torch.cat((fa["k_proj"][1], fa["v_proj"][1]), 0))
        self.const["final.kv_pe"] = cres(torch.cat((kpe @ fa["k_proj"][0].t(), torch.zeros(kpe.shape[0], 128)), 1))
        self._norm("norm_final", f"{D}.transformer.norm_final_attn", 256)
        for key, mod, cin, cout in (("up1", f"{D}.output_upscaling.0", 256, 64), ("up2", f"{D}.output_upscaling.3", 64, 32)):
            w = self.p.weight(mod, (cin, cout, 2, 2))
            b = self.p.bias(mod, cout)
            self._pack(key, _lin(w.permute(2, 3, 1, 0).reshape(4 * cout, cin)), b.repeat(4))
        self._norm("up_ln", f"{D}.output_upscaling.1", 64)
        for i in range(4):
            for j, (co, ci) in enumerate(((256, 256), (256, 256), (32, 256))):
                self._linear(f"hyper{i}.{j}", f"{D}.output_hypernetworks_mlps.{i}.layers.{j}", co, ci)
        for j, (co, ci) in enumerate(((256, 256), (256, 256), (4, 256))):
            self._linear(f"iou.{j}", f"{D}.iou_prediction_head.layers.{j}", co, ci)
        for j, (co, ci) in enumerate(((256, 256), (256, 256), (1, 256))):
            self.p.weight(f"{D}.pred_obj_score_head.layers.{j}", (co, ci)); self.p.bias(f"{D}.pred_obj_score_head.layers.{j}", co)
        del self.key_pe, self.sparse, self._sa_w, self._x_w, self.tokens

    def _refinement(self):
        if not self.use_refinement:
            self.refine_params = None
            return
        parts = []
        for j, k in enumerate(self.kernels):
            parts.append(self.p.tensor(f"refinement_layer.conv_branches.{j}.weight", (4, 1, k, k), "refine").reshape(-1))
            parts.append(self.p.tensor(f"refinement_layer.conv_branches.{j}.bias", (4,), "refine"))
        parts.append(self.p.tensor("refinement_layer.combiner_conv.weight", (1, 4 * len(self.kernels), 1, 1), "refine").reshape(-1))
        parts.append(self.p.tensor("refinement_layer.combiner_conv.bias", (1,), "refine"))
        self.refine_params = torch.cat([t.float() for t in parts]).to(self.device)


class Sam2Plan:

    def __init__(self, wt, B, stream, dynamic_multimask_via_stability=True, prompts=0, points=3, high_res=True, attn="16", mask_prompt=False,
                 multimask=False):
        self.wt, self.B, self.dt, self.dev = wt, B, wt.dtype, wt.device
        if attn not in ("16", "fp8") or (attn == "fp8" and not is16(wt.dtype)):
            raise ValueError("attn must be '16' or 'fp8' (fp8 needs an fp16 / bf16 plan)")
        self.av_fp8 = 1 if attn == "fp8" else 0
        self._ln1_stats, self._ln1_parts = None, 0
        self.P, self.K, self.want_high_res = prompts, points, high_res
        if prompts and not wt.prompt_ok:
            raise _lib.CvmiError("this checkpoint carries no sam_prompt_encoder tensors: box / point prompts are unavailable")
        if (mask_prompt or multimask) and not prompts:
            raise ValueError("mask_prompt / multimask need prompts > 0 (the learned-prompt wrapper always runs single-mask without a mask input)")
        if mask_prompt and not wt.mask_prompt_ok:
            raise _lib.CvmiError("this checkpoint carries no sam_prompt_encoder.mask_downscaling tensors: mask prompts are unavailable")
        self.mask_prompt, self.multimask = bool(mask_prompt), bool(multimask)
        self.plan = Plan(stream)
        self.pool = {}
        self.dynamic = dynamic_multimask_via_stability
        self.act_bytes = 0
        self._build()
        torch.cuda.synchronize()

    def buf(self, H, W, C, dtype=None, tag=None, zero=False, batch=None):
        dtype = self.dt if dtype is None else dtype
        batch = self.B if batch is None else batch
        key = (batch, H, W, C, dtype, tag)
        if tag is None or key not in self.pool:
            b = Buf(batch, H, W, C, dtype, self.dev, zero=zero)
            self.act_bytes += b.nbytes
            if tag is None:
                return b
            self.pool[key] = b
        return self.pool[key]

    def gemm(self, label, key, src, dst, act=ACT_NONE, res=None, kind="gemm", **kw):
        srcs = src if isinstance(src, list) else [(src, 0)]
        op_conv(self.plan, label, self.wt.pc[key], srcs, dst, act=act, res=res, kind=kind, **kw)

    def _build(self):
        wt, B = self.wt, self.B
        R = wt.image_size
        g = R // 4
        self.x_in = Buf(B, R, R, 3, self.dt, self.dev, zero=True)
        E = wt.hiera["embed_dim"]
        x = self.buf(g, g, E, F32)
        pos = wt.const["pos_embed"]
        self.plan.keep.append(pos)
        xs = Buf(B, g, g, 48, self.dt, self.dev)
        lib = _lib.load()
        op_call(self.plan, "s2d4", "stem", lib.cvmi_space_to_depth4, (self.x_in.t.data_ptr(), xs.t.data_ptr(), B, R, R, self.dt),
                keep=(self.x_in, xs), bytes_=2 * self.x_in.nbytes)
        op_conv(self.plan, "patch_embed", wt.pc["patch_embed"], [(xs.view(), 0)], x.view(), stride=1, pad=1, out_hw=(g, g),
                res=_ConstView(pos, E), res_mod=g * g, kind="stem")
        H = W = g
        stage_out = []
        for i, blk in enumerate(wt.blocks):
            x, H, W = self._block(i, blk, x, H, W)
            if i in wt.stage_ends:
                stage_out.append(x)
        self.stage_out = stage_out
        self._neck_decoder(stage_out)

    def _block(self, i, blk, x, H, W):
        wt, B = self.wt, self.B
        dim, dout, heads, ws = blk["dim"], blk["dim_out"], blk["heads"], blk["window"]
        hd = dout // heads
        gam, bet = wt.ln[f"b{i}.norm1"]
        Hp, Wp = (H, W) if ws == 0 else (-(-H // ws) * ws, -(-W // ws) * ws)
        padded = (Hp, Wp) != (H, W)
        if blk["q_pool"] and (ws == 0 or ws % 2 or Hp % 2 or Wp % 2):
            raise NotImplementedError("q-pool block needs an even window")
        tok_rows = not padded and (B * H * W) % 256 == 0
        tok_qkv = tok_rows and f"b{i}.qkv" in wt.tl
        if dim != dout and os.environ.get("CVMI_SAM_QKVTOK_TRANS", "1") == "0":
            tok_qkv = False
        tok_pool = tok_rows and dim != dout and f"b{i}.dimproj" in wt.tl and os.environ.get("CVMI_SAM_POOLFUSE", "1") != "0"
        if padded:
            xn = self.buf(Hp, Wp, dim, tag="xn_padded", zero=True)
            op_layernorm(self.plan, f"b{i}.norm1", x.view(), gam, bet, xn.view(), 1e-6, pad=(H, W, Hp, Wp))
        elif not tok_qkv or (dim != dout and not tok_pool):
            xn = self.buf(H, W, dim, tag="xn")
            op_layernorm(self.plan, f"b{i}.norm1", x.view(), gam, bet, xn.view(), 1e-6)
        parts = self._ln1_parts
        ln1_stats = self._ln1_stats if (self._ln1_stats is not None and self._ln1_stats.numel() == 2 * B * H * W * max(parts, 1)) else None
        self._ln1_stats, self._ln1_parts = None, 0
        if dim != dout:
            short = self.buf(H // 2, W // 2, dout, F32)
            if tok_pool:
                op_tok_linear_pool(self.plan, f"b{i}.dimproj_pool", wt.tl[f"b{i}.dimproj"], x.view(), short.view(), (gam, bet, 1e-6),
                                   stats_in=ln1_stats if parts == 0 else None)
            else:
                pj = self.buf(H, W, dout, F32, tag="dimproj")
                self.gemm(f"b{i}.dimproj", f"b{i}.dimproj", xn.view(), pj.view(), out_hw=(H, W) if padded else None)
                op_maxpool2(self.plan, f"b{i}.pool", pj.view(), short.view())
        else:
            short = x
        fuse_qkv = (tok_qkv and ws > 0 and f"b{i}.qkv_attn" in wt.tl and not self.av_fp8 and (ln1_stats is None or parts == 0)
                    and qkv_attn_supported(dim, dout, heads, ws, blk["q_pool"], self.dt, B * (Hp // ws) * (Wp // ws)))
        qkv = None if fuse_qkv else self.buf(Hp, Wp, 3 * dout, tag="qkv")
        if fuse_qkv:
            pass
        elif tok_qkv:
            op_tok_linear(self.plan, f"b{i}.qkv", wt.tl[f"b{i}.qkv"], x.view(), qkv.view(), ln=(gam, bet, 1e-6), stats_in=ln1_stats, stats_parts=parts)
        else:
            self.gemm(f"b{i}.qkv", f"b{i}.qkv", xn.view(), qkv.view())
        OH, OW = (H // 2, W // 2) if blk["q_pool"] else (H, W)
        OHp, OWp = (Hp // 2, Wp // 2) if blk["q_pool"] else (Hp, Wp)
        ao = self.buf(OHp, OWp, dout, tag="ao")
        es = ESIZE[self.dt]
        base = qkv.t.data_ptr() if qkv is not None else 0
        C3 = 3 * dout
        if fuse_qkv:
            nwin, pq = B * (H // ws) * (W // ws), wt.tl[f"b{i}.qkv_attn"]
            xv = x.view()
            nq = (ws // 2) ** 2 if blk["q_pool"] else ws * ws
            desc = make_attn_desc(q=None, k=None, v=None, o=ao.t.data_ptr(), q_sb=0, q_sh=hd, q_st=C3, k_sb=0, k_sh=hd, k_st=C3, v_sb=0, v_sh=hd, v_st=C3,
                                  o_sb=0, o_sh=hd, o_st=dout, B=nwin, heads=heads, Nq=nq, Nk=ws * ws, dqk=hd, dv=hd, scale=hd ** -0.5, dtype=self.dt,
                                  win=ws, grid_h=H, grid_w=W, q_pool=1 if blk["q_pool"] else 0, av_fp8=0, q_log2=1 if wt.q_log2 else 0,
                                  proj_x=xv.ptr, proj_ld=xv.ld, proj_K=dim, proj_w=pq.w.data_ptr(), proj_gamma=gam.data_ptr(), proj_beta=bet.data_ptr(),
                                  proj_eps=1e-6, proj_stats=ln1_stats.data_ptr() if ln1_stats is not None else None)
            rows = B * H * W
            op_attention(self.plan, f"b{i}.attn", desc, (x, ao, pq, gam, bet, ln1_stats), bytes_=rows * dim * 4 + ao.nbytes,
                         flops=2 * rows * C3 * dim + 4 * nwin * heads * nq * ws * ws * hd)
            self.plan.ops[-1] = (self.plan.ops[-1][0], "attn_window") + self.plan.ops[-1][2:]
        elif ws > 0:
            nwin = B * (Hp // ws) * (Wp // ws)
            nq = (ws // 2) ** 2 if blk["q_pool"] else ws * ws
            desc = make_attn_desc(q=base, k=base + dout * es, v=base + 2 * dout * es, o=ao.t.data_ptr(),
                                  q_sb=0, q_sh=hd, q_st=C3, k_sb=0, k_sh=hd, k_st=C3, v_sb=0, v_sh=hd, v_st=C3,
                                  o_sb=0, o_sh=hd, o_st=dout, B=nwin, heads=heads, Nq=nq, Nk=ws * ws, dqk=hd, dv=hd,
                                  scale=hd ** -0.5, dtype=self.dt, win=ws, grid_h=Hp, grid_w=Wp, q_pool=1 if blk["q_pool"] else 0, av_fp8=self.av_fp8,
                                  q_log2=1 if wt.q_log2 else 0)
            fl = 4 * nwin * heads * nq * ws * ws * hd
        else:
            N = H * W
            desc = make_attn_desc(q=base, k=base + dout * es, v=base + 2 * dout * es, o=ao.t.data_ptr(),
                                  q_sb=N * C3, q_sh=hd, q_st=C3, k_sb=N * C3, k_sh=hd, k_st=C3, v_sb=N * C3, v_sh=hd, v_st=C3,
                                  o_sb=N * dout, o_sh=hd, o_st=dout, B=B, heads=heads, Nq=N, Nk=N, dqk=hd, dv=hd,
                                  scale=hd ** -0.5, dtype=self.dt, win=0, grid_h=0, grid_w=0, q_pool=0, av_fp8=self.av_fp8, q_log2=1 if wt.q_log2 else 0)
            fl = 4 * B * heads * N * N * hd
        if not fuse_qkv:
            op_attention(self.plan, f"b{i}.attn", desc, (qkv, ao), bytes_=qkv.nbytes + ao.nbytes, flops=fl)
            self.plan.ops[-1] = (self.plan.ops[-1][0], "attn_global" if ws == 0 else "attn_window") + self.plan.ops[-1][2:]
        tok_out = not padded and (B * OH * OW) % 256 == 0
        fwd = (tok_out and f"b{i}.proj" in wt.tl and f"b{i}" not in wt.mlp and f"b{i}.fc1" in wt.tl
               and os.environ.get("CVMI_SAM_LNSTATS", "1") != "0")
        sparts = tok_linear_stats_parts(B * OH * OW, dout, dout) if fwd else 0
        stats = torch.empty(B * OH * OW, max(sparts, 1), 2, dtype=torch.float32, device=self.dev) if fwd else None
        if tok_out and f"b{i}.proj" in wt.tl:
            op_tok_linear(self.plan, f"b{i}.proj", wt.tl[f"b{i}.proj"], ao.view(), short.view(), residual=True, stats_out=stats, stats_eps=1e-6)
        else:
            self.gemm(f"b{i}.proj", f"b{i}.proj", ao.view(), short.view(), res=short.view(), out_hw=(OH, OW) if padded else None)
        x = short
        gam, bet = wt.ln[f"b{i}.norm2"]
        if f"b{i}" in wt.mlp:
            nxt = wt.blocks[i + 1] if i + 1 < len(wt.blocks) else None
            if nxt is not None and os.environ.get("CVMI_SAM_LNSTATS", "1") != "0" and f"b{i + 1}.qkv" in wt.tl and (B * OH * OW) % 256 == 0:
                self._ln1_stats = torch.empty(B * OH * OW, 2, dtype=torch.float32, device=self.dev)
            op_hiera_mlp(self.plan, f"b{i}.mlp", wt.mlp[f"b{i}"], x.view(), gam, bet, 1e-6, stats_out=self._ln1_stats, stats_eps=1e-6)
        else:
            hid = self.buf(OH, OW, 4 * dout, tag="hid")
            if tok_out and f"b{i}.fc1" in wt.tl:
                op_tok_linear(self.plan, f"b{i}.fc1", wt.tl[f"b{i}.fc1"], x.view(), hid.view(), ln=(gam, bet, 1e-6), act=ACT_GELU, stats_in=stats, stats_parts=sparts)
            else:
                xn2 = self.buf(OH, OW, dout, tag="xn")
                op_layernorm(self.plan, f"b{i}.norm2", x.view(), gam, bet, xn2.view(), 1e-6)
                self.gemm(f"b{i}.fc1", f"b{i}.fc1", xn2.view(), hid.view(), act=ACT_GELU)
            rs = None
            nxt_qkv = f"b{i + 1}.qkv" in wt.tl and i + 1 < len(wt.blocks) and wt.blocks[i + 1]["dim"] == dout
            if (nxt_qkv and tok_out and self.dt != F32 and row_stats_supported(B * OH * OW, dout, 4 * dout)
                    and os.environ.get("CVMI_SAM_LNSTATS", "1") != "0" and os.environ.get("CVMI_SAM_LNSTATS_FC2", "1") != "0"):
                rs = torch.empty(B * OH * OW, dout // 96, 2, dtype=torch.float32, device=self.dev)
                self._ln1_stats, self._ln1_parts = rs, dout // 96
            self.gemm(f"b{i}.fc2", f"b{i}.fc2", hid.view(), x.view(), res=x.view(), row_stats=rs)
        if i in self.wt.stage_ends and i != len(self.wt.blocks) - 1:
            pass
        return x, OH, OW

    def _neck_decoder(self, st):
        wt, B, dt = self.wt, self.B, self.dt
        R = wt.image_size
        f0, f1, fs = R // 4, R // 8, R // 16
        def cast(buf, tag):
            if dt == F32:
                return buf
            o = self.buf(buf.H, buf.W, buf.C, dt)
            op_cast(self.plan, f"cast.{tag}", buf.view(), o.view())
            return o
        feat_s0 = self.buf(f0, f0, 32)
        feat_s1 = self.buf(f1, f1, 64)
        fused = os.environ.get("CVMI_SAM_NECKCAST", "1") != "0"
        for key, src, dstb, tag in (("feat_s0", st[0], feat_s0, "s0"), ("feat_s1", st[1], feat_s1, "s1")):
            if fused and key in wt.tl and src.dtype == F32 and (B * src.H * src.W) % 256 == 0:
                op_tok_linear(self.plan, key, wt.tl[key], src.view(), dstb.view(), ln="cast", kind="neck")
            else:
                self.gemm(key, key, cast(src, tag).view(), dstb.view(), kind="neck")
        s2, s3 = cast(st[2], "s2"), cast(st[3], "s3")
        lib = _lib.load()
        NP = self.P
        NB = B * NP if NP else B
        P = fs * fs
        bufd = lambda *a, **k: self.buf(*a, batch=NB, **k)
        if not NP:
            keys = self.buf(fs, fs, 256, F32)
            dense = wt.const["dense"]
            self.gemm("embed", "embed", [(s2.view(), 0), (s3.view(), 1)], keys.view(), res=_ConstView(dense, 256), res_mod=fs * fs, kind="neck")
            T = wt.n_tok
            qn0 = Buf(B, 1, T, 256, dt, self.dev)
            qn0.t.copy_(wt.const["tokens"].to(TORCH_DTYPE[dt]).view(1, 1, T, 256).expand(B, 1, T, 256))
            tpe = lambda name, C_: dict(res=_ConstView(wt.const[name], C_), res_mod=T)
        else:
            emb = self.buf(fs, fs, 256, F32)
            self.gemm("embed", "embed_box", [(s2.view(), 0), (s3.view(), 1)], emb.view(), kind="neck")
            keys = bufd(fs, fs, 256, F32)
            self.share_l0 = is16(dt) and os.environ.get("CVMI_SAM_SHARE_L0", "1") != "0" and not self.mask_prompt
            if self.mask_prompt:
                self.mask_in = torch.zeros(NB, f0, f0, dtype=torch.float32, device=self.dev)
                kn0 = bufd(fs, fs, 256, tag="kn") if is16(dt) else None
                op_call(self.plan, "mask_prompt_embed", "decoder", lib.cvmi_mask_prompt_embed,
                        (self.mask_in.data_ptr(), emb.t.data_ptr(), wt.const["mask_down"].data_ptr(), keys.t.data_ptr(),
                         kn0.t.data_ptr() if kn0 is not None else None, dt if kn0 is not None else F16, B, NP, fs),
                        keep=(emb, keys, kn0), bytes_=NB * f0 * f0 * 4 + (B + NB) * P * 256 * 4 + (NB * P * 256 * 2 if kn0 is not None else 0),
                        flops=2 * NB * P * (16 * 4 + 16 * 16 + 256 * 16))
            elif not self.share_l0:
                op_call(self.plan, "repeat_embed", "decoder", lib.cvmi_repeat_images, (emb.t.data_ptr(), keys.t.data_ptr(), P * 256 * 4, B, NP),
                        keep=(emb, keys), bytes_=(B + NB) * P * 256 * 4)
            T = 6 + self.K
            self.coords = torch.zeros(NB, self.K, 2, dtype=torch.float32, device=self.dev)
            self.labels = torch.full((NB, self.K), -1, dtype=torch.int32, device=self.dev)
            tok0 = Buf(NB, 1, T, 256, F32, self.dev)
            qn0 = Buf(NB, 1, T, 256, dt, self.dev)
            op_call(self.plan, "prompt_tokens", "decoder", lib.cvmi_prompt_tokens,
                    (self.coords.data_ptr(), self.labels.data_ptr(), wt.const["gauss"].data_ptr(), wt.const["out_tokens"].data_ptr(),
                     wt.const["prompt_table"].data_ptr(), float(R), tok0.t.data_ptr(), qn0.t.data_ptr(), dt, NB, self.K, 6),
                    keep=(tok0, qn0), bytes_=NB * T * 256 * 6)
            npe = wt.pc["token_pe"].N
            pe_all = Buf(NB, 1, T, npe, dt, self.dev)
            self.gemm("token_pe", "token_pe", qn0.view(), pe_all.view(), kind="decoder")
            tpe = lambda name, C_: dict(res=pe_all.view(wt.pe_off[name][0], C_))
            self.tokens0 = tok0
        self.feat_s0, self.feat_s1, self.keys0 = feat_s0, feat_s1, keys
        q = Buf(NB, 1, T, 256, F32, self.dev, zero=True)

        def ln(label, key, src, dst, dst2=None):
            gam, bet = wt.ln[key]
            op_layernorm(self.plan, label, src.view(), gam, bet, dst.view(), 1e-5, dst2=dst2.view() if dst2 is not None else None)

        def attention(label, qb, q_off, kb, k_off, vb, v_off, ob, Nq, Nk, hd, q_bdiv=0, kv_bdiv=0):
            es = ESIZE[dt]
            desc = make_attn_desc(q=qb.t.data_ptr() + q_off * es, k=kb.t.data_ptr() + k_off * es, v=vb.t.data_ptr() + v_off * es, o=ob.t.data_ptr(),
                                  q_sb=Nq * qb.C, q_sh=hd, q_st=qb.C, k_sb=Nk * kb.C, k_sh=hd, k_st=kb.C, v_sb=Nk * vb.C, v_sh=hd, v_st=vb.C,
                                  o_sb=Nq * ob.C, o_sh=hd, o_st=ob.C, B=NB, heads=8, Nq=Nq, Nk=Nk, dqk=hd, dv=hd, scale=hd ** -0.5, dtype=dt,
                                  win=0, grid_h=0, grid_w=0, q_pool=0, q_bdiv=q_bdiv, kv_bdiv=kv_bdiv)
            op_attention(self.plan, label, desc, (qb, kb, vb, ob), flops=4 * NB * 8 * Nq * Nk * hd)
            self.plan.ops[-1] = (self.plan.ops[-1][0], "decoder") + self.plan.ops[-1][2:]

        dual = is16(dt)
        qn = bufd(1, T, 256, tag="qn")
        kn = bufd(fs, fs, 256, tag="kn")
        G = lambda *a, **k: self.gemm(*a, kind="decoder", **k)
        for l in (0, 1):
            p = f"l{l}"
            qkv = bufd(1, T, 768, tag="sa_qkv")
            if l == 0:
                G(f"{p}.sa.qkv", f"{p}.sa.qkv", qn0.view(), qkv.view())
            else:
                op_cast(self.plan, f"{p}.sa.cast", q.view(), qn.view())
                G(f"{p}.sa.qkv", f"{p}.sa.qkv", qn.view(), qkv.view(), **tpe(f"{p}.sa.qkv_pe", 768))
            ao = bufd(1, T, 256, tag="sa_ao")
            attention(f"{p}.sa.attn", qkv, 0, qkv, 256, qkv, 512, ao, T, T, 32)
            if l == 0:
                G(f"{p}.sa.out", f"{p}.sa.out", ao.view(), q.view())
            else:
                G(f"{p}.sa.out", f"{p}.sa.out", ao.view(), q.view(), res=q.view())
            ln(f"{p}.norm1", f"{p}.norm1", q, q)
            op_cast(self.plan, f"{p}.t2i.castq", q.view(), qn.view())
            share = l == 0 and NP and getattr(self, "share_l0", False)
            if share:
                kn_l = self.buf(fs, fs, 256, tag="kn_shared")
                op_cast(self.plan, f"{p}.t2i.castk", emb.view(), kn_l.view())
            else:
                kn_l = kn
                if not dual or (l == 0 and not self.mask_prompt):
                    op_cast(self.plan, f"{p}.t2i.castk", keys.view(), kn.view())
            tq = bufd(1, T, 128, tag="t2i_q")
            G(f"{p}.t2i.q", f"{p}.t2i.q", qn.view(), tq.view(), **tpe(f"{p}.t2i.q_pe", 128))
            kv = self.buf(fs, fs, 256, tag="t2i_kv_shared") if share else bufd(fs, fs, 256, tag="t2i_kv")
            G(f"{p}.t2i.kv", f"{p}.t2i.kv", kn_l.view(), kv.view(), res=_ConstView(wt.const[f"{p}.t2i.kv_pe"], 256), res_mod=P)
            ao2 = bufd(1, T, 128, tag="t2i_ao")
            attention(f"{p}.t2i.attn", tq, 0, kv, 0, kv, 128, ao2, T, P, 16, kv_bdiv=NP if share else 0)
            G(f"{p}.t2i.out", f"{p}.t2i.out", ao2.view(), q.view(), res=q.view())
            ln(f"{p}.norm2", f"{p}.norm2", q, q)
            op_cast(self.plan, f"{p}.mlp.cast", q.view(), qn.view())
            hid = bufd(1, T, 2048, tag="mlp_hid")
            G(f"{p}.mlp1", f"{p}.mlp1", qn.view(), hid.view(), act=ACT_RELU)
            G(f"{p}.mlp2", f"{p}.mlp2", hid.view(), q.view(), res=q.view())
            ln(f"{p}.norm3", f"{p}.norm3", q, q)
            op_cast(self.plan, f"{p}.i2t.castq", q.view(), qn.view())
            iq = self.buf(fs, fs, 128, tag="i2t_q_shared") if share else bufd(fs, fs, 128, tag="i2t_q")
            G(f"{p}.i2t.q", f"{p}.i2t.q", kn_l.view(), iq.view(), res=_ConstView(wt.const[f"{p}.i2t.q_pe"], 128), res_mod=P)
            ikv = bufd(1, T, 256, tag="i2t_kv")
            G(f"{p}.i2t.kv", f"{p}.i2t.kv", qn.view(), ikv.view(), **tpe(f"{p}.i2t.kv_pe", 256))
            ao3 = bufd(fs, fs, 128, tag="i2t_ao")
            attention(f"{p}.i2t.attn", iq, 0, ikv, 0, ikv, 128, ao3, P, T, 16, q_bdiv=NP if share else 0)
            if share:
                G(f"{p}.i2t.out", f"{p}.i2t.out", ao3.view(), keys.view(), res=emb.view(), res_mod=P, res_rep=NP)
            else:
                G(f"{p}.i2t.out", f"{p}.i2t.out", ao3.view(), keys.view(), res=keys.view())
            ln(f"{p}.norm4", f"{p}.norm4", keys, keys, dst2=kn if dual else None)
        op_cast(self.plan, "final.castq", q.view(), qn.view())
        if not dual:
            op_cast(self.plan, "final.castk", keys.view(), kn.view())
        tq = bufd(1, T, 128, tag="t2i_q")
        G("final.q", "final.q", qn.view(), tq.view(), **tpe("final.q_pe", 128))
        kv = bufd(fs, fs, 256, tag="t2i_kv")
        G("final.kv", "final.kv", kn.view(), kv.view(), res=_ConstView(wt.const["final.kv_pe"], 256), res_mod=P)
        ao2 = bufd(1, T, 128, tag="t2i_ao")
        attention("final.attn", tq, 0, kv, 0, kv, 128, ao2, T, P, 16)
        G("final.out", "final.out", ao2.view(), q.view(), res=q.view())
        ln("norm_final", "norm_final", q, q)
        self.tokens_out, self.keys_out = q, keys
        u1 = bufd(f1, f1, 64)
        G("up1", "up1", kn.view(), u1.view(), res=feat_s1.view(), shuffle_cout=64, res_rep=NP)
        gam, bet = wt.ln["up_ln"]
        op_layernorm(self.plan, "up_ln", u1.view(), gam, bet, u1.view(), 1e-6, act=ACT_GELU)
        u2 = bufd(f0, f0, 32)
        G("up2", "up2", u1.view(), u2.view(), res=feat_s0.view(), shuffle_cout=32, act=ACT_GELU, act_after_res=True, res_rep=NP)
        self.up = u2
        op_cast(self.plan, "heads.cast", q.view(), qn.view())
        hyper = Buf(NB, 1, 4, 32, F32, self.dev)
        for i in range(4):
            src = _RowsView(qn.t, NB, 256, ld=T * 256, offset=(2 + i) * 256, dtype=dt)
            h1 = bufd(1, 1, 256, tag="h1"); h2 = bufd(1, 1, 256, tag="h2")
            G(f"hyper{i}.0", f"hyper{i}.0", src, h1.view(), act=ACT_RELU)
            G(f"hyper{i}.1", f"hyper{i}.1", h1.view(), h2.view(), act=ACT_RELU)
            G(f"hyper{i}.2", f"hyper{i}.2", h2.view(), _RowsView(hyper.t, NB, 32, ld=128, offset=i * 32, dtype=F32))
        iou4 = Buf(NB, 1, 1, 4, F32, self.dev)
        src = _RowsView(qn.t, NB, 256, ld=T * 256, offset=256, dtype=dt)
        h1 = bufd(1, 1, 256, tag="h1"); h2 = bufd(1, 1, 256, tag="h2")
        G("iou.0", "iou.0", src, h1.view(), act=ACT_RELU)
        G("iou.1", "iou.1", h1.view(), h2.view(), act=ACT_RELU)
        G("iou.2", "iou.2", h2.view(), iou4.view(), act=ACT_SIGMOID)
        self.hyper, self.iou4 = hyper, iou4
        P0 = f0 * f0
        self.masks4 = torch.empty(NB, 4, f0, f0, dtype=torch.float32, device=self.dev)
        self.areas = torch.zeros(NB, 2, dtype=torch.int32, device=self.dev)
        NM = 3 if self.multimask else 1
        self.low_res = torch.empty(NB, NM, f0, f0, dtype=torch.float32, device=self.dev)
        self.iou = torch.empty(NB, NM, dtype=torch.float32, device=self.dev)
        self.sel = torch.zeros(NB, dtype=torch.int32, device=self.dev)
        op_call(self.plan, "hyper_masks", "tail", lib.cvmi_hyper_masks,
                (hyper.t.data_ptr(), 32, u2.t.data_ptr(), 32, dt, 32, self.masks4.data_ptr(), self.areas.data_ptr(), NB, P0, 0.05),
                keep=(hyper, u2), bytes_=NB * P0 * (32 * ESIZE[dt] + 16), flops=2 * NB * P0 * 128)
        if self.multimask:
            op_call(self.plan, "multimask_out", "tail", lib.cvmi_multimask_out,
                    (self.masks4.data_ptr(), iou4.t.data_ptr(), 4, self.low_res.data_ptr(), self.iou.data_ptr(), NB, P0), bytes_=NB * P0 * 24)
        else:
            op_call(self.plan, "select_mask", "tail", lib.cvmi_select_mask,
                    (self.masks4.data_ptr(), self.areas.data_ptr(), iou4.t.data_ptr(), 4, 1 if self.dynamic else 0, 0.98, self.low_res.data_ptr(),
                     self.iou.data_ptr(), self.sel.data_ptr(), NB, P0), bytes_=NB * P0 * 8)
        if not self.want_high_res:
            self.high_res = None
            return
        self.high_res = torch.empty(NB, NM, R, R, dtype=torch.float32, device=self.dev)
        if wt.refine_params is not None and not NP:
            import ctypes as C
            ks = (C.c_int * len(wt.kernels))(*wt.kernels)
            taps = sum(k * k for k in wt.kernels)
            op_call(self.plan, "upsample_refine", "tail", lib.cvmi_upsample_refine,
                    (self.low_res.data_ptr(), NB, f0, f0, self.high_res.data_ptr(), R, R, wt.refine_params.data_ptr(), ks, len(wt.kernels), 4),
                    keep=(ks,), bytes_=NB * (P0 + R * R) * 4, flops=2 * NB * R * R * 4 * taps)
        else:
            op_call(self.plan, "upsample", "tail", lib.cvmi_bilinear_f32,
                    (self.low_res.data_ptr(), NB * NM, f0, f0, self.high_res.data_ptr(), R, R, None, 0.0), bytes_=NB * NM * (P0 + R * R) * 4)

class _ConstView:

    def __init__(self, t, C):
        self.t, self.c = t, C

    ptr = property(lambda s: s.t.data_ptr())
    ld = property(lambda s: s.c)


class _RowsView:

    def __init__(self, t, rows, C, ld, offset, dtype):
        self.t, self.B, self.H, self.W, self.c, self._ld, self.off, self.dtype = t, rows, 1, 1, C, ld, offset, dtype

    ptr = property(lambda s: s.t.data_ptr() + s.off * s.t.element_size())
    ld = property(lambda s: s._ld)
```

include/cvmi355.h:

```cpp
#ifndef CVMI355_H
#define CVMI355_H

#include <stddef.h>
#include <stdint.h>

#ifdef __cplusplus
extern "C" {
#endif

#define CVMI_VERSION 126

typedef void* cvmi_stream_t;

enum { CVMI_F16 = 0, CVMI_F32 = 1, CVMI_BF16 = 2 };
enum { CVMI_ACT_NONE = 0, CVMI_ACT_SILU = 1, CVMI_ACT_RELU = 2, CVMI_ACT_GELU = 3, CVMI_ACT_SIGMOID = 4 };

int cvmi_version(void);
const char* cvmi_last_error(void);
const char* cvmi_last_kernel(void);
int cvmi_device_info(int device, int* out4);
enum { CVMI_DESC_CONV = 0, CVMI_DESC_C3K2 = 1, CVMI_DESC_DWPW = 2, CVMI_DESC_ATTN = 3 };
size_t cvmi_desc_size(int kind);

int cvmi_graph_begin(cvmi_stream_t stream);
int cvmi_graph_end(cvmi_stream_t stream, void** graph_exec_out);
int cvmi_graph_launch(void* graph_exec, cvmi_stream_t stream);
int cvmi_graph_destroy(void* graph_exec);

typedef struct cvmi_conv_desc {
  const void* x0; const void* x1;
  const void* w; const float* bias;
  const void* res;
  void* y;
  int x0_ld, x1_ld, res_ld, y_ld;
  int c0, c1;
  int up0, up1;
  int B, H, W;
  int OH, OW;
  int KH, KW, stride, pad;
  int N;
  int Kpad;
  int act;
  int dtype;
  int out_f32;
  int scalar_gather;
  int res_mod;
  int act_after_res;
  int shuffle_cout;
  int res_rep;
  float* row_stats;
} cvmi_conv_desc;
int cvmi_conv2d(const cvmi_conv_desc* d, cvmi_stream_t stream);

typedef struct {
  const void* x; void* y;
  const void *w0, *w1, *w2, *w3;
  const float *b0, *b1, *b2, *b3;
  int x_ld, y_ld, kpad0, kpad1, kpad2, kpad3;
  int B, H, W, c1, c, h, c2;
  int fuse_cv1, shortcut, dtype;
} cvmi_c3k2_desc;
int cvmi_c3k2_supported(int c1, int c, int h, int c2, int fuse_cv1, int dtype);
int cvmi_c3k2(const cvmi_c3k2_desc* d, cvmi_stream_t stream);

int cvmi_stem2_supported(int c0, int c1, int dtype);
int cvmi_stem2(const void* x, int x_ld, const void* w0, const float* b0, int kpad0, const void* w1, const float* b1, int kpad1,
               void* y, int y_ld, int B, int H2, int W2, int c0, int c1, int dtype, cvmi_stream_t stream);

typedef struct {
  const void* x; void* y;
  const void* wd; const float* bd;
  const void* w1; const float* b1;
  const void* w2; const float* b2;
  int x_ld, y_ld, kpad1, kpad2;
  int B, H, W, C, N1, N2;
  int dtype;
} cvmi_dwpw_desc;
int cvmi_dwpw_supported(int C, int N1, int N2, int dtype);
int cvmi_dwpw(const cvmi_dwpw_desc* d, cvmi_stream_t stream);

int cvmi_dwconv3x3(const void* x, int x_ld, const void* w, const float* bias, const void* res,
                   int res_ld, void* y, int y_ld, int B, int H, int W, int C, int act, int dtype,
                   cvmi_stream_t stream);

int cvmi_sppf_pool(void* buf, int ld, int B, int H, int W, int C, int dtype, cvmi_stream_t stream);

typedef struct cvmi_attn_desc {
  const void* q; const void* k; const void* v; void* o;
  long long q_sb, q_sh, q_st, k_sb, k_sh, k_st, v_sb, v_sh, v_st, o_sb, o_sh, o_st;
  int B, heads, Nq, Nk, dqk, dv;
  float scale;
  int dtype;
  int win, grid_h, grid_w;
  int q_pool;
  int q_bdiv, kv_bdiv;
  int av_fp8;
  int q_log2;
  const void* proj_x;
  const void* proj_w;
  const float* proj_gamma;
  const float* proj_beta;
  const float* proj_stats;
  int proj_ld, proj_K;
  float proj_eps;
} cvmi_attn_desc;
int cvmi_attention(const cvmi_attn_desc* d, cvmi_stream_t stream);

int cvmi_detect_decode(const void* const* box, const int* box_ld, const void* const* cls,
                       const int* cls_ld, const int* hs, const int* ws, const float* strides,
                       int nlevels, int B, int nc, int dtype, float* pred, float* best_score,
                       int* best_cls, int write_cls, cvmi_stream_t stream);

size_t cvmi_yolo_nms_workspace(int B, int A);
int cvmi_yolo_nms(const float* pred, int B, int nc, int A, float conf_thres, float iou_thres,
                  int max_det, float max_wh, float* out_det, int* out_idx, int* out_count,
                  void* workspace, cvmi_stream_t stream);
int cvmi_yolo_nms_best(const float* pred, const float* best_score, const int* best_cls, int B, int nc,
                       int A, float conf_thres, float iou_thres, int max_det, float max_wh,
                       float* out_det, int* out_idx, int* out_count, void* workspace,
                       cvmi_stream_t stream);

int cvmi_letterbox(const uint8_t* src, int H, int W, void* dst, int out_h, int out_w, int new_h,
                   int new_w, int top, int left, int dtype, int s2d, cvmi_stream_t stream);
int cvmi_letterbox_batch(const uint8_t* src, int B, int H, int W, void* dst, long long dst_image_stride, int out_h, int out_w,
                         int new_h, int new_w, int top, int left, int dtype, int s2d, cvmi_stream_t stream);
typedef struct cvmi_letterbox_row {
  long long src_byte_offset;
  int H, W, new_h, new_w, top, left;
} cvmi_letterbox_row;
int cvmi_letterbox_ragged(const uint8_t* src, long long src_bytes, const cvmi_letterbox_row* rows, int B, void* dst,
                          long long dst_image_stride, int out_h, int out_w, int dtype, int s2d, cvmi_stream_t stream);

int cvmi_nchw_to_nhwc(const void* src, int src_dtype, void* dst, int dst_dtype, int dst_ld, int B,
                      int C, int H, int W, cvmi_stream_t stream);
int cvmi_nhwc_to_nchw_f32(const void* src, int src_dtype, int src_ld, float* dst, int B, int C,
                          int H, int W, cvmi_stream_t stream);


int cvmi_layernorm(const void* x, int x_ld, int x_dtype, const float* gamma, const float* beta,
                   void* y, int y_ld, int y_dtype, long long rows, int C, float eps, int act,
                   int pad_h, int pad_w, int pad_hp, int pad_wp, cvmi_stream_t stream);
int cvmi_layernorm_dual(const void* x, int x_ld, const float* gamma, const float* beta, void* y, int y_ld, void* y2, int y2_ld,
                        int y2_dtype , long long rows, int C, float eps, cvmi_stream_t stream);

int cvmi_hiera_mlp_supported(int C);
size_t cvmi_hiera_mlp_packed_bytes(int C);
int cvmi_hiera_mlp(void* x, int x_ld, const float* gamma, const float* beta, float eps, const void* w_packed,
                   const float* b2, long long rows, int C, int dtype , cvmi_stream_t stream);
int cvmi_hiera_mlp_stats(void* x, int x_ld, const float* gamma, const float* beta, float eps, const void* w_packed, const float* b2,
                         long long rows, int C, int dtype, float* ln_stats_out, float ln_stats_eps, cvmi_stream_t stream);

int cvmi_tok_linear_supported(int K);
size_t cvmi_tok_linear_packed_bytes(int K, int N);
int cvmi_tok_linear_format(int K);
int cvmi_tok_linear(const void* in, int in_ld, int in_f32_layernorm, const float* gamma, const float* beta, float eps,
                    const void* w_packed, void* out, int out_ld, int out_f32_residual, long long rows, int K, int N, int act,
                    int dtype , cvmi_stream_t stream);

int cvmi_tok_linear_stats(const void* in, int in_ld, int in_f32_layernorm, const float* gamma, const float* beta, float eps,
                          const void* w_packed, void* out, int out_ld, int out_f32_residual, long long rows, int K, int N, int act,
                          int dtype, const float* ln_stats_in, int ln_stats_in_parts, float* ln_stats_out, float ln_stats_eps,
                          cvmi_stream_t stream);
int cvmi_tok_linear_stats_parts(long long rows, int K, int N);

int cvmi_tok_linear_pool(const void* in, int in_ld, const float* gamma, const float* beta, float eps, const void* w_packed, void* out,
                         int out_ld, int B, int H, int W, int K, int N, int dtype, cvmi_stream_t stream);
int cvmi_tok_linear_pool_stats(const void* in, int in_ld, const float* gamma, const float* beta, float eps, const void* w_packed, void* out,
                               int out_ld, int B, int H, int W, int K, int N, int dtype, const float* ln_stats_in, cvmi_stream_t stream);

int cvmi_maxpool2x2(const void* x, int x_ld, void* y, int y_ld, int B, int H, int W, int C, int dtype,
                    cvmi_stream_t stream);

int cvmi_space_to_depth4(const void* x, void* y, int B, int H, int W, int dtype, cvmi_stream_t stream);

int cvmi_cast(const void* x, int x_ld, int x_dtype, void* y, int y_ld, int y_dtype, long long rows, int C,
              cvmi_stream_t stream);

int cvmi_prompt_tokens(const float* coords, const int* labels, const float* gauss, const float* out_tokens,
                       const float* table, float image_size, float* tokens_f32, void* tokens_lp, int dtype,
                       int n, int K, int T0, cvmi_stream_t stream);

int cvmi_repeat_images(const void* src, void* dst, long long bytes_per_image, int B, int rep, cvmi_stream_t stream);

int cvmi_hyper_masks(const float* hyper, int hyper_ld, const void* up, int up_ld, int up_dtype, int C,
                     float* masks, int* areas, int B, int P, float delta, cvmi_stream_t stream);
int cvmi_select_mask(const float* masks, const int* areas, const float* iou, int iou_ld, int dynamic,
                     float thresh, float* low_res, float* iou_out, int* sel, int B, int P,
                     cvmi_stream_t stream);

int cvmi_multimask_out(const float* masks, const float* iou, int iou_ld, float* low_res3, float* iou3, int n, int P,
                       cvmi_stream_t stream);

#define CVMI_MASK_PROMPT_PARAMS 4684
int cvmi_mask_prompt_embed(const float* mask, const float* emb, const float* params, float* keys, void* keys_lp, int lp_dtype,
                           int B, int rep, int fs, cvmi_stream_t stream);

int cvmi_bilinear_f32(const float* x, int N, int h, int w, float* y, int H, int W, uint8_t* mask_u8,
                      float thresh, cvmi_stream_t stream);

int cvmi_mask_postprocess(const float* x, int N, int h, int w, int H, int W, float thresh, uint8_t* mask_u8,
                          int* extent, cvmi_stream_t stream);
int cvmi_mask_postprocess_sizes(const float* x, int N, int h, int w, const int* sizes, float thresh, uint8_t* mask_u8, int* extent,
                                cvmi_stream_t stream);
int cvmi_mask_postprocess_rects_dev(const float* x, int N, int h, int w, const int* rects_dev, long long plane_stride, float thresh,
                                    uint8_t* mask_u8, int* extent, cvmi_stream_t stream);

#define CVMI_MASK_CC_TILE 64
size_t cvmi_mask_cc_workspace(int N, int h, int w);
int cvmi_mask_components(const float* x, int N, int h, int w, float thresh, int* labels, int* areas, void* workspace,
                         cvmi_stream_t stream);
int cvmi_mask_fill_small(const float* x, int N, int h, int w, float thresh, float max_hole_area, float max_sprinkle_area, float* y,
                         void* workspace, cvmi_stream_t stream);

int cvmi_mask_extent(const uint8_t* mask, int N, int H, int W, int* extent, cvmi_stream_t stream);

int cvmi_upsample_refine(const float* low, int N, int h, int w, float* high, int H, int W,
                         const float* params, const int* ks, int nk, int ic, cvmi_stream_t stream);

int cvmi_sam2_transform(const uint8_t* src, int H, int W, void* dst, int R, int dst_dtype,
                        cvmi_stream_t stream);
int cvmi_sam2_transform_batch(const uint8_t* src, int B, int H, int W, void* dst, int R, int dst_dtype, int swap_rb,
                              cvmi_stream_t stream);
int cvmi_sam2_transform_rects(const uint8_t* src, long long src_image_stride, int H, int W, const int* rects, int B, void* dst, int R,
                              int dst_dtype, int swap_rb, cvmi_stream_t stream);
int cvmi_sam2_transform_rects_dev(const uint8_t* src, long long src_image_stride, int H, int W, const int* rects_dev, int B, void* dst, int R,
                                  int dst_dtype, int swap_rb, cvmi_stream_t stream);
typedef struct cvmi_sam2_src_row {
  long long src_byte_offset;
  int H, W;
  int x0, y0, w, h;
} cvmi_sam2_src_row;
int cvmi_sam2_transform_srcs(const uint8_t* src, long long src_bytes, const cvmi_sam2_src_row* rows, int B, void* dst, int R, int dst_dtype,
                             int swap_rb, cvmi_stream_t stream);

#define CVMI_GLUE_MAX_DET 320
#define CVMI_GLUE_INFO_HEAD 40
#define CVMI_GLUE_CLASS_NOT_CLUSTERED 1
#define CVMI_GLUE_CLASS_JUNCTION 2
#define CVMI_GLUE_CLASS_TEXT 4
#define CVMI_GLUE_CLASS_NON_COMPONENT 8
#define CVMI_GLUE_BOX_EXPANDED 1
#define CVMI_GLUE_BOX_DROPPED 2
enum {
  CVMI_GLUE_REASON = 0,
  CVMI_GLUE_DECISION = 1,
  CVMI_GLUE_APPLIED = 2,
  CVMI_GLUE_LINK = 3,
  CVMI_GLUE_CLUSTERS = 4,
  CVMI_GLUE_MAIN_SIZE = 5,
  CVMI_GLUE_MAIN_TEXT = 6,
  CVMI_GLUE_MAIN_ID = 7,
  CVMI_GLUE_MAIN_FIRST = 8,
  CVMI_GLUE_TOTAL = 9,
  CVMI_GLUE_COMPONENT_TYPE = 10,
  CVMI_GLUE_TEXT_TYPE = 11,
  CVMI_GLUE_PADDING = 12,
  CVMI_GLUE_BASIS_SET = 13,
  CVMI_GLUE_PADDED_SET = 14,
  CVMI_GLUE_FINAL_SET = 15,
  CVMI_GLUE_BASIS = 16,
  CVMI_GLUE_PADDED = 24,
  CVMI_GLUE_FINAL = 28
};
enum { CVMI_GLUE_REASON_NONE = 0, CVMI_GLUE_REASON_NO_ELEMENTS = 1, CVMI_GLUE_REASON_TOO_LARGE = 2, CVMI_GLUE_REASON_INVALID = 3 };
enum { CVMI_GLUE_DECISION_UNKNOWN = 0, CVMI_GLUE_DECISION_NO_ELEMENTS = 1, CVMI_GLUE_DECISION_SCORED = 2, CVMI_GLUE_DECISION_FALLBACK = 3 };
int cvmi_stage2_crop(const float* det, const int* count, int B, int max_det, int H0, int W0, float gain, int pad_x, int pad_y,
                     double stage2_iou, int padding, const uint8_t* class_flags, int n_flags, int* kept_idx, int* kept_count, int* boxes,
                     int* adj_boxes, int* window, int* info, cvmi_stream_t stream);


int cvmi_node_prepare(const uint8_t* src, int N, const int* sizes, const int* boxes, const int* box_start, uint8_t* emptied,
                      uint8_t* resized, cvmi_stream_t stream);

int cvmi_enhance_lines(const uint8_t* src, int N, const int* sizes, uint8_t* dst, unsigned long long* sums, cvmi_stream_t stream);

size_t cvmi_contours_workspace(int N, const int* sizes);
int cvmi_external_contours(uint8_t* planes, const unsigned long long* sums, int N, const int* sizes, int binarize, void* workspace,
                           size_t workspace_bytes, int cap_contours, int cap_points, int* counts, int* info, long long* area2,
                           int* points, cvmi_stream_t stream);

size_t cvmi_node_connect_workspace(int N, int C);
int cvmi_node_connect(const int* info, const int* points, int C, int P, const int* boxes, int N, const int* box_start, const int* pair_start,
                      void* workspace, size_t workspace_bytes, int* first, long long* moments, cvmi_stream_t stream);


int cvmi_segment_circuit(const uint8_t* src, size_t src_bytes, int N, const long long* planes, int red_channel, const int* rects,
                         const int* box_start, uint8_t* dst, unsigned long long* sums, cvmi_stream_t stream);

size_t cvmi_contour_hits_workspace(int N, int C);
int cvmi_contour_hits(const int* info, const int* points, int C, int P, const int* boxes, int N, const int* box_start, const int* pair_start,
                      void* workspace, size_t workspace_bytes, int* first, cvmi_stream_t stream);

#ifdef __cplusplus
}
#endif
#endif
```

Measured before the change: 378.0 images/s.

## Fuse Hiera attention output projection into the fused MLP kernel

Adds a proj+MLP fused kernel path for Hiera blocks with C=144/288. It computes the attention output projection (ao·Wp + bp) plus residual inside the MLP kernel before the LayerNorm and MLP, streaming the proj weights through the same LDS slots. This removes a separate proj GEMM launch and one fp32 residual write and read of x per block. In exchange, per-block register and LDS pressure rises, weights are packed a second time, and the path is only taken when the layout is unpadded and contiguous.

```diff
diff --git a/circuitvision_amd/_lib.py b/circuitvision_amd/_lib.py
--- a/circuitvision_amd/_lib.py
+++ b/circuitvision_amd/_lib.py
@@ -62,6 +62,10 @@
         ("proj_x", C.c_void_p), ("proj_w", C.c_void_p), ("proj_gamma", C.c_void_p), ("proj_beta", C.c_void_p), ("proj_stats", C.c_void_p),
         ("proj_ld", C.c_int), ("proj_K", C.c_int), ("proj_eps", C.c_float),
     ]
+
+
+class MlpProj(C.Structure):
+    _fields_ = [("ao", C.c_void_p), ("w_packed", C.c_void_p), ("bp", C.c_void_p), ("ao_ld", C.c_int)]
 
 
 class LetterboxRow(C.Structure):
@@ -112,7 +116,8 @@
     "cvmi_hiera_mlp_supported": (_i, [_i]),
     "cvmi_hiera_mlp_packed_bytes": (C.c_size_t, [_i]),
     "cvmi_hiera_mlp": (_i, [_vp, _i, _vp, _vp, _f, _vp, _vp, C.c_longlong, _i, _i, _vp]),
-    "cvmi_hiera_mlp_stats": (_i, [_vp, _i, _vp, _vp, _f, _vp, _vp, C.c_longlong, _i, _i, _vp, _f, _vp]),
+    "cvmi_hiera_mlp_proj_packed_bytes": (C.c_size_t, [_i]),
+    "cvmi_hiera_mlp_stats": (_i, [_vp, _i, _vp, _vp, _f, _vp, _vp, C.c_longlong, _i, _i, _vp, _f, _vp, C.POINTER(MlpProj)]),
     "cvmi_tok_linear_supported": (_i, [_i]),
     "cvmi_tok_linear_packed_bytes": (C.c_size_t, [_i, _i]),
     "cvmi_tok_linear_format": (_i, [_i]),
diff --git a/circuitvision_amd/csrc/hiera_mlp.hip b/circuitvision_amd/csrc/hiera_mlp.hip
--- a/circuitvision_amd/csrc/hiera_mlp.hip
+++ b/circuitvision_amd/csrc/hiera_mlp.hip
@@ -33,21 +33,23 @@
   static constexpr int LDS = SLOTS * CHB + 1024;
 };
 
-template <int C, int VAR = 0>
-__global__ __launch_bounds__((MlpCfg<C, VAR>::NW * 64), (MlpCfg<C, VAR>::WPS)) void hiera_mlp_kernel(float* __restrict__ x, int x_ld, const float* __restrict__ gamma,
-                                                                                      const float* __restrict__ beta, float eps,
-                                                                                      const char* __restrict__ wp, const float* __restrict__ b2,
-                                                                                      long long rows, float* __restrict__ stats_out, float stats_eps) {
+template <int C, int VAR> struct MlpWave {
   using Cfg = MlpCfg<C, VAR>;
-  constexpr int KS = Cfg::KS, KS1 = Cfg::KS1, NT = Cfg::NT, NCH = Cfg::NCH, FR = Cfg::FR, CHB = Cfg::CHB, NW = Cfg::NW, CNT = Cfg::CNT, SLOTS = Cfg::SLOTS;
-  extern __shared__ __attribute__((aligned(16))) char smem[];
-  const int tid = threadIdx.x, wv = __builtin_amdgcn_readfirstlane(tid >> 6), lane = tid & 63;
-  const int lr = lane & 31, lh = lane >> 5;
-  const long long row_raw = ((long long)blockIdx.x * NW + wv) * 32 + lr;
-  const bool row_ok = row_raw < rows;
-  float* const xr = x + (row_ok ? row_raw : rows - 1) * (long long)x_ld;
-
-  auto issue_chunk = [&](int j) {
+  char* smem;
+  const char* wp;
+  int wv, lane, lr, lh;
+  long long row_raw, row_clamped;
+  bool row_ok;
+  __device__ __forceinline__ MlpWave(char* smem_, const char* wp_, long long rows) : smem(smem_), wp(wp_) {
+    const int tid = threadIdx.x;
+    wv = __builtin_amdgcn_readfirstlane(tid >> 6), lane = tid & 63;
+    lr = lane & 31, lh = lane >> 5;
+    row_raw = ((long long)blockIdx.x * Cfg::NW + wv) * 32 + lr;
+    row_ok = row_raw < rows;
+    row_clamped = row_ok ? row_raw : rows - 1;
+  }
+  __device__ __forceinline__ void issue_chunk(int j) const {
+    constexpr int FR = Cfg::FR, CHB = Cfg::CHB, NW = Cfg::NW, CNT = Cfg::CNT, SLOTS = Cfg::SLOTS;
     const char* src = wp + (size_t)j * CHB + lane * 16;
     char* dst = smem + (j % SLOTS) * CHB;
 #pragma unroll
@@ -57,8 +59,9 @@
       __builtin_amdgcn_global_load_lds((const __attribute__((address_space(1))) void*)(src + (size_t)(real ? fi : 0) * 1024),
                                        (__attribute__((address_space(3))) void*)(real ? dst + fi * 1024 : smem + SLOTS * CHB), 16, 0, 0);
     }
-  };
-  auto issue_piece = [&](int st, int f) {
+  }
+  __device__ __forceinline__ void issue_piece(int st, int f) const {
+    constexpr int KS1 = Cfg::KS1, NT = Cfg::NT, NCH = Cfg::NCH, FR = Cfg::FR, CHB = Cfg::CHB, NW = Cfg::NW, SLOTS = Cfg::SLOTS;
     const int lo = st < 0 ? 2 * NT : 0, hi = st == NCH - 1 ? 2 * NT : FR;
     const char* src = wp + ((long long)st * FR + KS1) * 1024 + lane * 16;
     char* dst = smem + ((st + SLOTS) % SLOTS) * CHB;
@@ -66,62 +69,69 @@
     const bool real = fi >= lo && fi < hi;
     __builtin_amdgcn_global_load_lds((const __attribute__((address_space(1))) void*)(src + (long long)(real ? fi : lo) * 1024),
                                      (__attribute__((address_space(3))) void*)(real ? dst + fi * 1024 : smem + SLOTS * CHB), 16, 0, 0);
-  };
-  auto issue_stage = [&](int st) {
-#pragma unroll
-    for (int f = 0; f < CNT; ++f) issue_piece(st, f);
-  };
-  if constexpr (VAR == 2) {
-#pragma unroll
-    for (int st = -1; st < SLOTS - 1; ++st) issue_stage(st);
-  } else {
-#pragma unroll
-    for (int j = 0; j < SLOTS - 1; ++j) issue_chunk(j);
-  }
-
-  u32x4 xn[KS1];
-  {
-    float v[KS][8];
-    float s = 0.f;
-#pragma unroll
-    for (int k = 0; k < KS; ++k) {
-      const f32x4 a = *reinterpret_cast<const f32x4*>(xr + 16 * k + 8 * lh), b = *reinterpret_cast<const f32x4*>(xr + 16 * k + 8 * lh + 4);
-#pragma unroll
-      for (int e = 0; e < 4; ++e) { v[k][e] = a[e]; v[k][4 + e] = b[e]; s += a[e] + b[e]; }
-    }
-    s += __shfl_xor(s, 32);
-    const float mean = s / (float)C;
-    float q = 0.f;
-#pragma unroll
-    for (int k = 0; k < KS; ++k)
-#pragma unroll
-      for (int e = 0; e < 8; ++e) { const float d = v[k][e] - mean; q += d * d; }
-    q += __shfl_xor(q, 32);
-    const float rstd = 1.0f / sqrtf(q / (float)C + eps);
-#pragma unroll
-    for (int k = 0; k < KS; ++k) {
-      const float* gp = gamma + 16 * k + 8 * lh;
-      const float* bp = beta + 16 * k + 8 * lh;
-      const f32x4 g0 = *reinterpret_cast<const f32x4*>(gp), g1 = *reinterpret_cast<const f32x4*>(gp + 4);
-      const f32x4 b0 = *reinterpret_cast<const f32x4*>(bp), b1 = *reinterpret_cast<const f32x4*>(bp + 4);
-      f16x8 h;
-#pragma unroll
-      for (int e = 0; e < 4; ++e) {
-        h[e] = (f16)((v[k][e] - mean) * rstd * g0[e] + b0[e]);
-        h[4 + e] = (f16)((v[k][4 + e] - mean) * rstd * g1[e] + b1[e]);
-      }
-      xn[k] = __builtin_bit_cast(u32x4, h);
-    }
-    const u32x4 one = {lh == 0 ? CVMI_ONE16X2 : 0u, 0u, 0u, 0u};
-    xn[KS] = one;
-  }
-
-  f32x16 yacc[NT];
-#pragma unroll
-  for (int t = 0; t < NT; ++t)
-#pragma unroll
-    for (int r = 0; r < 16; ++r) yacc[t][r] = 0.f;
-
+  }
+  __device__ __forceinline__ void issue_stage(int st) const {
+#pragma unroll
+    for (int f = 0; f < Cfg::CNT; ++f) issue_piece(st, f);
+  }
+  __device__ __forceinline__ void issue_first() const {
+    if constexpr (VAR == 2) {
+#pragma unroll
+      for (int st = -1; st < Cfg::SLOTS - 1; ++st) issue_stage(st);
+    } else {
+#pragma unroll
+      for (int j = 0; j < Cfg::SLOTS - 1; ++j) issue_chunk(j);
+    }
+  }
+};
+
+template <int C, int VAR>
+__device__ __forceinline__ void mlp_ln_fragments(const float* xr, int lh, const float* __restrict__ gamma, const float* __restrict__ beta, float eps,
+                                                 u32x4 (&xn)[MlpCfg<C, VAR>::KS1]) {
+  constexpr int KS = MlpCfg<C, VAR>::KS;
+  float v[KS][8];
+  float s = 0.f;
+#pragma unroll
+  for (int k = 0; k < KS; ++k) {
+    const f32x4 a = *reinterpret_cast<const f32x4*>(xr + 16 * k + 8 * lh), b = *reinterpret_cast<const f32x4*>(xr + 16 * k + 8 * lh + 4);
+#pragma unroll
+    for (int e = 0; e < 4; ++e) { v[k][e] = a[e]; v[k][4 + e] = b[e]; s += a[e] + b[e]; }
+  }
+  s += __shfl_xor(s, 32);
+  const float mean = s / (float)C;
+  float q = 0.f;
+#pragma unroll
+  for (int k = 0; k < KS; ++k)
+#pragma unroll
+    for (int e = 0; e < 8; ++e) { const float d = v[k][e] - mean; q += d * d; }
+  q += __shfl_xor(q, 32);
+  const float rstd = 1.0f / sqrtf(q / (float)C + eps);
+#pragma unroll
+  for (int k = 0; k < KS; ++k) {
+    const float* gp = gamma + 16 * k + 8 * lh;
+    const float* bp = beta + 16 * k + 8 * lh;
+    const f32x4 g0 = *reinterpret_cast<const f32x4*>(gp), g1 = *reinterpret_cast<const f32x4*>(gp + 4);
+    const f32x4 b0 = *reinterpret_cast<const f32x4*>(bp), b1 = *reinterpret_cast<const f32x4*>(bp + 4);
+    f16x8 h;
+#pragma unroll
+    for (int e = 0; e < 4; ++e) {
+      h[e] = (f16)((v[k][e] - mean) * rstd * g0[e] + b0[e]);
+      h[4 + e] = (f16)((v[k][4 + e] - mean) * rstd * g1[e] + b1[e]);
+    }
+    xn[k] = __builtin_bit_cast(u32x4, h);
+  }
+  const u32x4 one = {lh == 0 ? CVMI_ONE16X2 : 0u, 0u, 0u, 0u};
+  xn[KS] = one;
+}
+
+template <int C, int VAR>
+__device__ __forceinline__ void mlp_chunk_loop(const MlpWave<C, VAR>& w, u32x4 (&xn)[MlpCfg<C, VAR>::KS1], f32x16 (&yacc)[MlpCfg<C, VAR>::NT]) {
+  using Cfg = MlpCfg<C, VAR>;
+  constexpr int KS1 = Cfg::KS1, NT = Cfg::NT, NCH = Cfg::NCH, FR = Cfg::FR, CHB = Cfg::CHB, CNT = Cfg::CNT, SLOTS = Cfg::SLOTS;
+  char* const smem = w.smem;
+  const int lane = w.lane;
+  auto issue_stage = [&](int st) { w.issue_stage(st); };
+  auto issue_chunk = [&](int j) { w.issue_chunk(j); };
   if constexpr (VAR == 2) {
     static_assert(SLOTS == 2, "two stages in LDS");
     constexpr int PF = 6;
@@ -256,10 +266,18 @@
       }
     }
   }
-
+}
+
+template <int C, int VAR, bool PROJ>
+__device__ __forceinline__ void mlp_epilogue(const MlpWave<C, VAR>& w, float* xr, f32x16 (&yacc)[MlpCfg<C, VAR>::NT], const float* __restrict__ b2,
+                                             const float* __restrict__ bp, float* __restrict__ stats_out, float stats_eps) {
+  constexpr int NT = MlpCfg<C, VAR>::NT;
+  const int lr = w.lr, lh = w.lh;
+  const bool row_ok = w.row_ok;
+  const long long row_raw = w.row_raw;
   ShiftedSums st;
   if (stats_out) {
-    const float o0 = row_ok ? xr[0] + (yacc[0][0] + b2[0]) : 0.f;
+    const float o0 = row_ok ? xr[0] + (yacc[0][0] + (PROJ ? bp[0] + b2[0] : b2[0])) : 0.f;
     st.shift = __shfl(o0, lr);
   }
   if (row_ok) {
@@ -269,7 +287,8 @@
       for (int g = 0; g < 4; ++g) {
         const int c0 = 32 * t + 8 * g + 4 * lh;
         if (c0 < C) {
-          const f32x4 bb = *reinterpret_cast<const f32x4*>(b2 + c0);
+          f32x4 bb = *reinterpret_cast<const f32x4*>(b2 + c0);
+          if constexpr (PROJ) bb += *reinterpret_cast<const f32x4*>(bp + c0);
           f32x4 o = *reinterpret_cast<const f32x4*>(xr + c0);
 #pragma unroll
           for (int e = 0; e < 4; ++e) o[e] += yacc[t][4 * g + e] + bb[e];
@@ -282,6 +301,27 @@
     const float2 mr = shifted_mean_rstd(st.shift, row_sum<2>(st.s), row_sum<2>(st.q), (float)C, stats_eps);
     if (row_ok && lh == 0) *reinterpret_cast<float2*>(stats_out + 2 * row_raw) = mr;
   }
+}
+
+template <int C, int VAR = 0>
+__global__ __launch_bounds__((MlpCfg<C, VAR>::NW * 64), (MlpCfg<C, VAR>::WPS)) void hiera_mlp_kernel(float* __restrict__ x, int x_ld, const float* __restrict__ gamma,
+                                                                                      const float* __restrict__ beta, float eps,
+                                                                                      const char* __restrict__ wp, const float* __restrict__ b2,
+                                                                                      long long rows, float* __restrict__ stats_out, float stats_eps) {
+  using Cfg = MlpCfg<C, VAR>;
+  extern __shared__ __attribute__((aligned(16))) char smem[];
+  const MlpWave<C, VAR> w(smem, wp, rows);
+  float* const xr = x + w.row_clamped * (long long)x_ld;
+  w.issue_first();
+  u32x4 xn[Cfg::KS1];
+  mlp_ln_fragments<C, VAR>(xr, w.lh, gamma, beta, eps, xn);
+  f32x16 yacc[Cfg::NT];
+#pragma unroll
+  for (int t = 0; t < Cfg::NT; ++t)
+#pragma unroll
+    for (int r = 0; r < 16; ++r) yacc[t][r] = 0.f;
+  mlp_chunk_loop<C, VAR>(w, xn, yacc);
+  mlp_epilogue<C, VAR, false>(w, xr, yacc, b2, nullptr, stats_out, stats_eps);
 }
 
 template <int C, int VAR = 0>
@@ -300,6 +340,8 @@
 
 }
 
+#include "proj_mlp.hpp"
+
 #ifndef CVMI_OPERAND_BF16
 extern "C" int cvmi_hiera_mlp_supported(int C) { return C == 144 || C == 288; }
 
@@ -308,23 +350,30 @@
   const size_t fr = (size_t)(C / 16 + 1) + 2 * (size_t)((C + 31) / 32);
   return (size_t)(4 * C / 32) * fr * 1024;
 }
+extern "C" size_t cvmi_hiera_mlp_proj_packed_bytes(int C) {
+  if (!cvmi_hiera_mlp_supported(C)) return 0;
+  return (size_t)((C + 31) / 32) * (size_t)(C / 16) * 1024 + cvmi_hiera_mlp_packed_bytes(C);
+}
 extern "C" int cvmi_hiera_mlp_stats_bf16(void* x, int x_ld, const float* gamma, const float* beta, float eps, const void* w_packed, const float* b2,
-                                         long long rows, int C, int dtype, float* ln_stats_out, float ln_stats_eps, cvmi_stream_t stream_);
+                                         long long rows, int C, int dtype, float* ln_stats_out, float ln_stats_eps, cvmi_stream_t stream_,
+                                         const cvmi_mlp_proj* proj);
 #endif
 
 extern "C" int CVMI_ENTRY(cvmi_hiera_mlp_stats)(void* x, int x_ld, const float* gamma, const float* beta, float eps, const void* w_packed, const float* b2,
-                                                long long rows, int C, int dtype, float* ln_stats_out, float ln_stats_eps, cvmi_stream_t stream_) {
+                                                long long rows, int C, int dtype, float* ln_stats_out, float ln_stats_eps, cvmi_stream_t stream_,
+                                                const cvmi_mlp_proj* proj) {
 #ifndef CVMI_OPERAND_BF16
-  if (dtype == CVMI_BF16) return cvmi_hiera_mlp_stats_bf16(x, x_ld, gamma, beta, eps, w_packed, b2, rows, C, dtype, ln_stats_out, ln_stats_eps, stream_);
+  if (dtype == CVMI_BF16) return cvmi_hiera_mlp_stats_bf16(x, x_ld, gamma, beta, eps, w_packed, b2, rows, C, dtype, ln_stats_out, ln_stats_eps, stream_, proj);
 #endif
   CVMI_CHECK(dtype == CVMI_T16, "hiera_mlp: dtype must be CVMI_F16 or CVMI_BF16");
-  CVMI_CHECK(x && gamma && beta && w_packed && b2 && rows > 0, "hiera_mlp: bad arguments");
+  CVMI_CHECK(x && gamma && beta && (w_packed || proj) && b2 && rows > 0, "hiera_mlp: bad arguments");
   CVMI_CHECK(C == 144 || C == 288, "hiera_mlp: C=%d is not built (144, 288)", C);
   CVMI_CHECK(x_ld >= C && x_ld % 4 == 0 && (((uintptr_t)x | (uintptr_t)gamma | (uintptr_t)beta | (uintptr_t)w_packed | (uintptr_t)b2) & 15) == 0 &&
                  ((uintptr_t)ln_stats_out & 7) == 0,
              "hiera_mlp: pointers / ld must be 16-byte aligned");
   hipStream_t s = (hipStream_t)stream_;
   float* xf = (float*)x;
+  if (proj) return proj_mlp_dispatch(xf, x_ld, proj, gamma, beta, eps, b2, rows, C, s, ln_stats_out, ln_stats_eps);
   if (C == 144) return launch_mlp<144, 1>(xf, x_ld, gamma, beta, eps, w_packed, b2, rows, s, ln_stats_out, ln_stats_eps);
   const char* const pipe = getenv("CVMI_MLP_PIPE");
   if (pipe && !(atoi(pipe) & 2)) return launch_mlp<288, 0>(xf, x_ld, gamma, beta, eps, w_packed, b2, rows, s, ln_stats_out, ln_stats_eps);
@@ -333,5 +382,5 @@
 
 extern "C" int CVMI_ENTRY(cvmi_hiera_mlp)(void* x, int x_ld, const float* gamma, const float* beta, float eps, const void* w_packed, const float* b2,
                                           long long rows, int C, int dtype, cvmi_stream_t stream_) {
-  return CVMI_ENTRY(cvmi_hiera_mlp_stats)(x, x_ld, gamma, beta, eps, w_packed, b2, rows, C, dtype, nullptr, 0.f, stream_);
-}
+  return CVMI_ENTRY(cvmi_hiera_mlp_stats)(x, x_ld, gamma, beta, eps, w_packed, b2, rows, C, dtype, nullptr, 0.f, stream_, nullptr);
+}
diff --git a/circuitvision_amd/csrc/proj_mlp.hpp b/circuitvision_amd/csrc/proj_mlp.hpp
--- /dev/null
+++ b/circuitvision_amd/csrc/proj_mlp.hpp
@@ -0,0 +1,162 @@
+#pragma once
+
+namespace {
+
+template <int C, int VAR> struct ProjCfg {
+  using M = MlpCfg<C, VAR>;
+  static_assert(M::SLOTS == 2, "the slot hand-over below is written for two slots");
+  static constexpr int KS = M::KS, NT = M::NT;
+  static constexpr int TP = M::FR / KS;
+  static constexpr int NPP = (NT + TP - 1) / TP;
+  static constexpr int BYTES = NT * KS * 1024;
+  static constexpr int slot(int p) { return ((VAR == 2 ? 0 : 1) + NPP - 1 - p) % 2; }
+  static constexpr int tiles(int p) { return p == NPP - 1 ? NT - TP * (NPP - 1) : TP; }
+  static_assert(TP >= 1 && NPP >= 2 && tiles(NPP - 1) >= 1 && TP * KS <= M::FR, "a piece fits a slot");
+};
+
+template <int C, int VAR, int P>
+__device__ __forceinline__ void proj_piece(const char* buf, const u32x4 (&af)[MlpCfg<C, VAR>::KS], f32x16 (&yacc)[MlpCfg<C, VAR>::NT]) {
+  using PC = ProjCfg<C, VAR>;
+  constexpr int KS = PC::KS, NF = PC::tiles(P) * KS, PF = 6;
+  static_assert(NF >= PF, "ring");
+  u32x4 ring[PF];
+  const unsigned lbase = (unsigned)(size_t)((const __attribute__((address_space(3))) char*)buf);
+#pragma unroll
+  for (int f = 0; f < PF; ++f) asm volatile("ds_read_b128 %0, %1 offset:%2" : "=v"(ring[f]) : "v"(lbase), "i"(f * 1024));
+#pragma unroll
+  for (int f = 0; f < NF; ++f) {
+    const int t = PC::TP * P + f / KS, s = f % KS;
+    ring_wait(ring[f % PF], (NF - 1 - f) < (PF - 1) ? (NF - 1 - f) : (PF - 1));
+    if constexpr (VAR == 2) {
+      if (s == 0) asm volatile(CVMI_MFMA_ASM " %0, %1, %2, 0" : "=a"(yacc[t]) : "v"(ring[f % PF]), "v"(af[s]));
+      else asm volatile(CVMI_MFMA_ASM " %0, %1, %2, %0" : "+a"(yacc[t]) : "v"(ring[f % PF]), "v"(af[s]));
+    } else {
+      yacc[t] = CVMI_MFMA_32X32X16(__builtin_bit_cast(f16x8, ring[f % PF]), __builtin_bit_cast(f16x8, af[s]), yacc[t], 0, 0, 0);
+    }
+    if (f + PF < NF) asm volatile("ds_read_b128 %0, %1 offset:%2" : "=v"(ring[f % PF]) : "v"(lbase), "i"((f + PF) * 1024));
+  }
+}
+
+template <int C, int VAR>
+__global__ __launch_bounds__((MlpCfg<C, VAR>::NW * 64), (MlpCfg<C, VAR>::WPS)) void proj_mlp_kernel(float* __restrict__ x, int x_ld, const f16* __restrict__ ao, int ao_ld,
+                                                                                     const char* __restrict__ wp, const float* __restrict__ bp,
+                                                                                     const float* __restrict__ gamma, const float* __restrict__ beta, float eps,
+                                                                                     const float* __restrict__ b2, long long rows,
+                                                                                     float* __restrict__ stats_out, float stats_eps) {
+  using Cfg = MlpCfg<C, VAR>;
+  using PC = ProjCfg<C, VAR>;
+  constexpr int KS = Cfg::KS, KS1 = Cfg::KS1, NT = Cfg::NT, CHB = Cfg::CHB, NW = Cfg::NW, NPP = PC::NPP;
+  extern __shared__ __attribute__((aligned(16))) char smem[];
+  const MlpWave<C, VAR> w(smem, wp + PC::BYTES, rows);
+  const int lh = w.lh;
+  float* const xr = x + w.row_clamped * (long long)x_ld;
+  const f16* const ar = ao + w.row_clamped * (long long)ao_ld;
+
+  auto issue_proj = [&](auto pc) {
+    constexpr int p = decltype(pc)::value;
+    tok_issue_chunk<PC::tiles(p) * KS, NW>(wp + (size_t)p * PC::TP * KS * 1024, smem + PC::slot(p) * CHB, w.wv, w.lane);
+  };
+  issue_proj(std::integral_constant<int, 0>{});
+  u32x4 af[KS];
+#pragma unroll
+  for (int s = 0; s < KS; ++s) af[s] = *reinterpret_cast<const u32x4*>(ar + 16 * s + 8 * lh);
+  f32x16 yacc[NT];
+  if constexpr (VAR != 2) {
+#pragma unroll
+    for (int t = 0; t < NT; ++t)
+#pragma unroll
+      for (int r = 0; r < 16; ++r) yacc[t][r] = 0.f;
+  }
+  static_for<0, NPP>([&](auto pc) {
+    constexpr int p = decltype(pc)::value;
+    asm volatile("s_waitcnt vmcnt(0)" ::: "memory");
+    __syncthreads();
+    if constexpr (p + 1 < NPP) issue_proj(std::integral_constant<int, p + 1>{});
+    else if constexpr (VAR == 2) w.issue_stage(-1);
+    else w.issue_chunk(0);
+    proj_piece<C, VAR, p>(smem + PC::slot(p) * CHB + w.lane * 16, af, yacc);
+  });
+  if constexpr (VAR == 2) {
+    __syncthreads();
+    w.issue_stage(0);
+    asm volatile("s_nop 15" : "+a"(yacc[NT - 1]));
+  }
+
+  u32x4 xn[KS1];
+  {
+    constexpr int LNG = 2;
+    float v[NT][16];
+    float s = 0.f;
+    const float *xp = xr + 4 * lh, *pp = bp + 4 * lh;
+#pragma unroll
+    for (int t = 0; t < NT; ++t) {
+      if (t % LNG == 0 && t > 0) asm volatile("" : "+v"(xp), "+v"(pp) : "v"(s));
+#pragma unroll
+      for (int g = 0; g < 4; ++g)
+        if (32 * t + 8 * g < C) {
+          const int c0 = 32 * t + 8 * g;
+          const f32x4 xv = *reinterpret_cast<const f32x4*>(xp + c0), pv = *reinterpret_cast<const f32x4*>(pp + c0);
+#pragma unroll
+          for (int e = 0; e < 4; ++e) {
+            v[t][4 * g + e] = xv[e] + (yacc[t][4 * g + e] + pv[e]);
+            s += v[t][4 * g + e];
+          }
+        }
+    }
+    s += __shfl_xor(s, 32);
+    const float mean = s / (float)C;
+    float q = 0.f;
+#pragma unroll
+    for (int k = 0; k < 2 * KS; ++k)
+#pragma unroll
+      for (int e = 0; e < 4; ++e) { const float d = v[k >> 2][4 * (k & 3) + e] - mean; q += d * d; }
+    q += __shfl_xor(q, 32);
+    const float rstd = 1.0f / sqrtf(q / (float)C + eps);
+    const float *gp = gamma + 4 * lh, *tp = beta + 4 * lh;
+#pragma unroll
+    for (int k = 0; k < KS; ++k) {
+      const int t = k >> 1, h = k & 1;
+      if (k % (2 * LNG) == 0 && k > 0) asm volatile("" : "+v"(gp), "+v"(tp) : "v"(xn[k - 1]));
+      const int c0 = 32 * t + 16 * h;
+      const f32x4 g0 = *reinterpret_cast<const f32x4*>(gp + c0), g1 = *reinterpret_cast<const f32x4*>(gp + c0 + 8);
+      const f32x4 b0 = *reinterpret_cast<const f32x4*>(tp + c0), b1 = *reinterpret_cast<const f32x4*>(tp + c0 + 8);
+      f16x8 hv;
+#pragma unroll
+      for (int e = 0; e < 4; ++e) {
+        hv[e] = (f16)((v[t][8 * h + e] - mean) * rstd * g0[e] + b0[e]);
+        hv[4 + e] = (f16)((v[t][8 * h + 4 + e] - mean) * rstd * g1[e] + b1[e]);
+      }
+      xn[k] = __builtin_bit_cast(u32x4, hv);
+    }
+    xn[KS] = tok_bias_fragment(lh);
+  }
+
+  asm volatile("s_waitcnt vmcnt(0)" ::: "memory");
+  mlp_chunk_loop<C, VAR>(w, xn, yacc);
+  mlp_epilogue<C, VAR, true>(w, xr, yacc, b2, bp, stats_out, stats_eps);
+}
+
+template <int C, int VAR>
+int launch_proj_mlp(float* x, int x_ld, const cvmi_mlp_proj* pj, const float* gamma, const float* beta, float eps, const float* b2, long long rows, hipStream_t s,
+                    float* stats_out, float stats_eps) {
+  using Cfg = MlpCfg<C, VAR>;
+  static hipError_t attr = hipFuncSetAttribute(reinterpret_cast<const void*>(&proj_mlp_kernel<C, VAR>), hipFuncAttributeMaxDynamicSharedMemorySize, Cfg::LDS);
+  CVMI_HIP(attr);
+  const long long per = (long long)Cfg::NW * 32;
+  cvmi_note_kernel("proj_mlp_kernel<%d, %d>", C, VAR);
+  hipLaunchKernelGGL((proj_mlp_kernel<C, VAR>), dim3((unsigned)((rows + per - 1) / per)), dim3(Cfg::NW * 64), Cfg::LDS, s, x, x_ld, (const f16*)pj->ao, pj->ao_ld,
+                     (const char*)pj->w_packed, pj->bp, gamma, beta, eps, b2, rows, stats_out, stats_eps);
+  CVMI_LAUNCH_CHECK();
+  return 0;
+}
+
+int proj_mlp_dispatch(float* x, int x_ld, const cvmi_mlp_proj* pj, const float* gamma, const float* beta, float eps, const float* b2, long long rows, int C,
+                      hipStream_t s, float* stats_out, float stats_eps) {
+  CVMI_CHECK(pj->ao && pj->w_packed && pj->bp, "proj_mlp: needs ao, the packed weights and bp");
+  CVMI_CHECK((((uintptr_t)pj->ao | (uintptr_t)pj->w_packed | (uintptr_t)pj->bp) & 15) == 0, "proj_mlp: ao / weights / bp are not aligned to 16 bytes");
+  CVMI_CHECK(pj->ao_ld >= C && pj->ao_ld % 8 == 0, "proj_mlp: ao_ld=%d must be >= C and a multiple of 8", pj->ao_ld);
+  if (C == 144) return launch_proj_mlp<144, 1>(x, x_ld, pj, gamma, beta, eps, b2, rows, s, stats_out, stats_eps);
+  return launch_proj_mlp<288, 2>(x, x_ld, pj, gamma, beta, eps, b2, rows, s, stats_out, stats_eps);
+}
+
+}
diff --git a/circuitvision_amd/engine.py b/circuitvision_amd/engine.py
--- a/circuitvision_amd/engine.py
+++ b/circuitvision_amd/engine.py
@@ -486,21 +486,26 @@
     return is16(dtype) and bool(_lib.load().cvmi_hiera_mlp_supported(C_))
 
 
+def _mlp_chunks(w1, b1, w2, td):
+    Hd, C_ = w1.shape
+    assert Hd == 4 * C_ and tuple(w2.shape) == (C_, Hd) and C_ % 16 == 0
+    ks1, nt, nch = C_ // 16 + 1, (C_ + 31) // 32, Hd // 32
+    b_hi = b1.to(td).float()
+    b_lo = (b1 - b_hi).to(td).float()
+    w1x = torch.cat((w1, b_hi[:, None], b_lo[:, None], torch.zeros(Hd, 14)), 1)
+    f1 = w1x.view(nch, 32, ks1, 2, 8).permute(0, 2, 3, 1, 4)
+    w2p = torch.zeros(nt * 32, Hd)
+    w2p[:C_] = w2
+    f2 = w2p.view(nt, 32, nch, 2, 2, 2, 4).permute(2, 0, 3, 5, 1, 4, 6)
+    return torch.cat((f1.reshape(nch, -1), f2.reshape(nch, -1)), 1).contiguous()
+
+
 class PackedHieraMlp:
 
     def __init__(self, w1, b1, w2, b2, device="cuda", dtype=F16):
         td = TORCH_DTYPE[dtype]
         Hd, C_ = w1.shape
-        assert Hd == 4 * C_ and tuple(w2.shape) == (C_, Hd) and C_ % 16 == 0
-        ks1, nt, nch = C_ // 16 + 1, (C_ + 31) // 32, Hd // 32
-        b_hi = b1.to(td).float()
-        b_lo = (b1 - b_hi).to(td).float()
-        w1x = torch.cat((w1, b_hi[:, None], b_lo[:, None], torch.zeros(Hd, 14)), 1)
-        f1 = w1x.view(nch, 32, ks1, 2, 8).permute(0, 2, 3, 1, 4)
-        w2p = torch.zeros(nt * 32, Hd)
-        w2p[:C_] = w2
-        f2 = w2p.view(nt, 32, nch, 2, 2, 2, 4).permute(2, 0, 3, 5, 1, 4, 6)
-        packed = torch.cat((f1.reshape(nch, -1), f2.reshape(nch, -1)), 1).contiguous()
+        packed = _mlp_chunks(w1, b1, w2, td)
         assert packed.numel() * 2 == _lib.load().cvmi_hiera_mlp_packed_bytes(C_)
         self.w = packed.to(td).to(device)
         self.bias = b2.float().contiguous().to(device)
@@ -508,21 +513,68 @@
         self.param_bytes = 2 * Hd * C_ * 2
 
 
-def op_hiera_mlp(plan, label, pm, x, gamma, beta, eps=1e-6, stats_out=None, stats_eps=1e-6):
-    lib = _lib.load()
+def proj_mlp_k_order(C_):
+    n = torch.arange(C_)
+    k = n % 16
+    return n - k + 8 * ((k & 7) >> 2) + 4 * (k >> 3) + (k & 3)
+
+
+class PackedProjMlp:
+
+    def __init__(self, wp, bp, w1, b1, w2, b2, device="cuda", dtype=F16):
+        td = TORCH_DTYPE[dtype]
+        Hd, C_ = w1.shape
+        assert tuple(wp.shape) == (C_, C_) and bp.numel() == C_ and b2.numel() == C_
+        nt, ks = (C_ + 31) // 32, C_ // 16
+        wpp = torch.zeros(nt * 32, C_)
+        wpp[:C_] = wp
+        fp = wpp.view(nt, 32, ks, 2, 8).permute(0, 2, 3, 1, 4)
+        packed = torch.cat((fp.reshape(-1), _mlp_chunks(w1[:, proj_mlp_k_order(C_)], b1, w2, td).reshape(-1)))
+        assert packed.numel() * 2 == _lib.load().cvmi_hiera_mlp_proj_packed_bytes(C_)
+        self.w = packed.to(td).to(device)
+        self.bias = torch.cat((bp.float(), b2.float())).contiguous().to(device)
+        self.C, self.dtype = C_, dtype
+        self.param_bytes = (C_ * C_ + 2 * Hd * C_) * 2
+
+    def unpack(self):
+        C_ = self.C
+        nt, ks, ks1, nch = (C_ + 31) // 32, C_ // 16, C_ // 16 + 1, 4 * C_ // 32
+        w, bias = self.w.cpu().float().reshape(-1), self.bias.cpu()
+        npj = nt * ks * 512
+        wp = w[:npj].view(nt, ks, 2, 32, 8).permute(0, 3, 1, 2, 4).reshape(nt * 32, C_)
+        ch = w[npj:].view(nch, -1)
+        f1 = ch[:, :ks1 * 512].reshape(nch, ks1, 2, 32, 8).permute(0, 3, 1, 2, 4).reshape(4 * C_, C_ + 16)
+        w1 = torch.zeros(4 * C_, C_)
+        w1[:, proj_mlp_k_order(C_)] = f1[:, :C_]
+        f2 = ch[:, ks1 * 512:].reshape(nch, nt, 2, 2, 32, 2, 4).permute(1, 4, 0, 2, 5, 3, 6).reshape(nt * 32, 4 * C_)
+        assert not wp[C_:].any() and not f2[C_:].any() and not f1[:, C_ + 2:].any()
+        return dict(wp=wp[:C_].clone(), bp=bias[:C_].clone(), w1=w1, b1=f1[:, C_] + f1[:, C_ + 1], w2=f2[:C_].clone(), b2=bias[C_:].clone())
+
+
+def op_hiera_mlp(plan, label, pm, x, gamma, beta, eps=1e-6, stats_out=None, stats_eps=1e-6, proj=None):
+    lib = _lib.load()
+    if proj is not None:
+        pm, ao = proj[0], _as_rows(proj[1])
     assert x.dtype == F32 and x.c == pm.C and x.c0 == 0
     rows = x.B * x.H * x.W
     assert stats_out is None or (stats_out.dtype == torch.float32 and stats_out.numel() == 2 * rows and stats_out.is_contiguous()), label
-    args = (x.ptr, x.ld, gamma.data_ptr(), beta.data_ptr(), float(eps), pm.w.data_ptr(), pm.bias.data_ptr(), rows, pm.C, pm.dtype,
+    desc, b2 = None, pm.bias.data_ptr()
+    if proj is not None:
+        assert ao.rows == rows and ao.C == pm.C and ao.dtype == pm.dtype, label
+        desc = _lib.MlpProj(ao=ao.ptr, w_packed=pm.w.data_ptr(), bp=pm.bias.data_ptr(), ao_ld=ao.ld)
+        b2 += 4 * pm.C
+    args = (x.ptr, x.ld, gamma.data_ptr(), beta.data_ptr(), float(eps), None if proj is not None else pm.w.data_ptr(), b2, rows, pm.C, pm.dtype,
             stats_out.data_ptr() if stats_out is not None else None, float(stats_eps))
-    plan.keep.append((pm, x, gamma, beta, stats_out))
+    plan.keep.append((pm, x, gamma, beta, stats_out, proj, desc))
     sp0, fn = plan.sptr, lib.cvmi_hiera_mlp_stats
-
-    def thunk(sp=None):
-        sp = sp0 if sp is None else sp
-        _lib.check(fn(*args, sp), label)
-
-    plan.add(label, "mlp_fused", thunk, rows * pm.C * 8, 2 * rows * 2 * 4 * pm.C * pm.C)
+    pdesc = C.byref(desc) if desc is not None else None
+
+    def thunk(sp=None):
+        sp = sp0 if sp is None else sp
+        _lib.check(fn(*args, sp, pdesc), label)
+
+    plan.add(label, "mlp_fused", thunk, rows * pm.C * (8 + (ESIZE[pm.dtype] if proj is not None else 0)),
+             2 * rows * 2 * 4 * pm.C * pm.C + (2 * rows * pm.C * pm.C if proj is not None else 0))
 
 
 def tok_linear_supported(K, dtype, rows):
diff --git a/circuitvision_amd/sam2.py b/circuitvision_amd/sam2.py
--- a/circuitvision_amd/sam2.py
+++ b/circuitvision_amd/sam2.py
@@ -9,7 +9,7 @@
 
 from . import _lib
 from ._lib import ACT_GELU, ACT_NONE, ACT_RELU, ACT_SIGMOID, BF16, F16, F32
-from .engine import (ESIZE, TORCH_DTYPE, is16, Buf, PackedConv, PackedHieraMlp, PackedQkvAttn, PackedTokLinear, Plan, Rows, hiera_mlp_supported, make_attn_desc, op_attention,
+from .engine import (ESIZE, TORCH_DTYPE, is16, Buf, PackedConv, PackedHieraMlp, PackedProjMlp, PackedQkvAttn, PackedTokLinear, Plan, Rows, hiera_mlp_supported, make_attn_desc, op_attention,
                      op_call, op_cast, op_conv, op_hiera_mlp, op_layernorm, op_maxpool2, op_tok_linear, op_tok_linear_pool, require_gpu, row_stats_supported,
                      qkv_attn_supported, tok_linear_stats_parts, tok_linear_supported)
 
@@ -244,6 +244,10 @@
                                                    self.p.weight(f"{b}.mlp.layers.1", (dim_out, 4 * dim_out)), self.p.bias(f"{b}.mlp.layers.1", dim_out),
                                                    self.device, self.dtype)
                 self.param_bytes += self.mlp[f"b{i}"].param_bytes
+                self.mlp[f"b{i}.projmlp"] = PackedProjMlp(self.p.weight(f"{b}.attn.proj", (dim_out, dim_out)), self.p.bias(f"{b}.attn.proj", dim_out),
+                                                          self.p.weight(f"{b}.mlp.layers.0", (4 * dim_out, dim_out)), self.p.bias(f"{b}.mlp.layers.0", 4 * dim_out),
+                                                          self.p.weight(f"{b}.mlp.layers.1", (dim_out, 4 * dim_out)), self.p.bias(f"{b}.mlp.layers.1", dim_out),
+                                                          self.device, self.dtype)
             else:
                 self._linear(f"b{i}.fc1", f"{b}.mlp.layers.0", 4 * dim_out, dim_out, tok=True)
                 self._linear(f"b{i}.fc2", f"{b}.mlp.layers.1", dim_out, 4 * dim_out)
@@ -546,7 +550,10 @@
                and os.environ.get("CVMI_SAM_LNSTATS", "1") != "0")
         sparts = tok_linear_stats_parts(B * OH * OW, dout, dout) if fwd else 0
         stats = torch.empty(B * OH * OW, max(sparts, 1), 2, dtype=torch.float32, device=self.dev) if fwd else None
-        if tok_out and f"b{i}.proj" in wt.tl:
+        fuse_proj = (f"b{i}.projmlp" in wt.mlp and not padded and ao.view().ld == dout and os.environ.get("CVMI_SAM_PROJMLP", "1") != "0")
+        if fuse_proj:
+            pass
+        elif tok_out and f"b{i}.proj" in wt.tl:
             op_tok_linear(self.plan, f"b{i}.proj", wt.tl[f"b{i}.proj"], ao.view(), short.view(), residual=True, stats_out=stats, stats_eps=1e-6)
         else:
             self.gemm(f"b{i}.proj", f"b{i}.proj", ao.view(), short.view(), res=short.view(), out_hw=(OH, OW) if padded else None)
@@ -556,7 +563,8 @@
             nxt = wt.blocks[i + 1] if i + 1 < len(wt.blocks) else None
             if nxt is not None and os.environ.get("CVMI_SAM_LNSTATS", "1") != "0" and f"b{i + 1}.qkv" in wt.tl and (B * OH * OW) % 256 == 0:
                 self._ln1_stats = torch.empty(B * OH * OW, 2, dtype=torch.float32, device=self.dev)
-            op_hiera_mlp(self.plan, f"b{i}.mlp", wt.mlp[f"b{i}"], x.view(), gam, bet, 1e-6, stats_out=self._ln1_stats, stats_eps=1e-6)
+            op_hiera_mlp(self.plan, f"b{i}.mlp", wt.mlp[f"b{i}"], x.view(), gam, bet, 1e-6, stats_out=self._ln1_stats, stats_eps=1e-6,
+                         proj=(wt.mlp[f"b{i}.projmlp"], ao.view()) if fuse_proj else None)
         else:
             hid = self.buf(OH, OW, 4 * dout, tag="hid")
             if tok_out and f"b{i}.fc1" in wt.tl:
diff --git a/include/cvmi355.h b/include/cvmi355.h
--- a/include/cvmi355.h
+++ b/include/cvmi355.h
@@ -8,7 +8,7 @@
 extern "C" {
 #endif
 
-#define CVMI_VERSION 126
+#define CVMI_VERSION 127
 
 typedef void* cvmi_stream_t;
 
@@ -147,8 +147,16 @@
 size_t cvmi_hiera_mlp_packed_bytes(int C);
 int cvmi_hiera_mlp(void* x, int x_ld, const float* gamma, const float* beta, float eps, const void* w_packed,
                    const float* b2, long long rows, int C, int dtype , cvmi_stream_t stream);
+typedef struct {
+  const void* ao;
+  const void* w_packed;
+  const float* bp;
+  int ao_ld;
+} cvmi_mlp_proj;
+size_t cvmi_hiera_mlp_proj_packed_bytes(int C);
 int cvmi_hiera_mlp_stats(void* x, int x_ld, const float* gamma, const float* beta, float eps, const void* w_packed, const float* b2,
-                         long long rows, int C, int dtype, float* ln_stats_out, float ln_stats_eps, cvmi_stream_t stream);
+                         long long rows, int C, int dtype, float* ln_stats_out, float ln_stats_eps, cvmi_stream_t stream,
+                         const cvmi_mlp_proj* proj);
 
 int cvmi_tok_linear_supported(int K);
 size_t cvmi_tok_linear_packed_bytes(int K, int N);
```

Result: faster. 386.9 images/s, median of 6 (+2.3%).
